# marcin119a/vae-los-angeles

Measured on AMD Instinct MI355X. Metric: training samples/sec, MultiModalVAE batch 65536, higher is better.
Workload: dtype bf16

## Files before the change

### include/mmvae_hip.h

```cpp
#ifndef MMVAE_HIP_H
#define MMVAE_HIP_H
#include <stdint.h>

#ifdef __cplusplus
extern "C" {
#endif

#define MMVAE_OK 0
#define MMVAE_ERR_ARG (-1)
#define MMVAE_ERR_DTYPE (-2)

enum { MMVAE_F32 = 0, MMVAE_BF16 = 1 };
enum { MMVAE_PREC_F32 = 0, MMVAE_PREC_BF16 = 1 };
enum { MMVAE_PRO_NONE = 0, MMVAE_PRO_BN_RELU_DROP = 1, MMVAE_PRO_BN_BWD_APPLY = 2 };
enum { MMVAE_EPI_STORE = 0, MMVAE_EPI_RELU_MASK = 1, MMVAE_EPI_BN_BWD = 2, MMVAE_EPI_LOSS_MSE = 3, MMVAE_EPI_LOSS_BCE_LOGIT = 4 };
enum { MMVAE_ACT_NONE = 0, MMVAE_ACT_RELU = 1, MMVAE_ACT_SIGMOID = 2 };

#define MMVAE_TILE 128

int mmvae_abi_version(void);
int mmvae_set_tuning(int32_t key, int32_t value);

typedef struct {
    const float* src; void* dst;
// ... 87 lines not shown
} mmvae_fuse_fwd_args;
int mmvae_fuse_reparam_fwd(const mmvae_fuse_fwd_args* args, void* stream);

typedef struct {
    int32_t B, L, n_mod;
    const float* g_mu; const float* g_lv;
    const float* dz; const float* dz2; const float* dz3; int64_t lddz;
    const float* eps; const float* logvar;
    float* d_heads; int64_t ld_heads;
    float* d_table; const int64_t* site; int32_t S;
    void* d_heads_lp; int64_t ld_heads_lp;
    int32_t table_copies;
} mmvae_fuse_bwd_args;
#define MMVAE_TABLE_COPIES 8
int mmvae_fuse_reparam_bwd(const mmvae_fuse_bwd_args* args, void* stream);

int mmvae_embed_proj_fwd(int32_t S, int32_t E, int32_t L, const float* emb, const float* w, const float* b, float* table, void* stream);
int mmvae_embed_proj_bwd(int32_t S, int32_t E, int32_t L, const float* emb, const float* w, const float* d_table, int32_t table_copies,
                         float* d_emb, float* d_w, float* d_b, void* stream);
typedef struct {
    int32_t B, L, n_mod;
    const float* head; int64_t ld_head;
    const float* table; const int64_t* site; int32_t S;
    float* latent;
    void* z; int32_t z_dtype; int64_t ldz;
} mmvae_fuse_mean_fwd_args;
int mmvae_fuse_mean_fwd(const mmvae_fuse_mean_fwd_args* args, void* stream);
typedef struct {
    int32_t B, L, n_mod;
    const float* dz; int64_t lddz;
    const float* g_latent;
    float* d_head; int64_t ld_head;
    void* d_head_lp; int64_t ld_head_lp;
    float* d_table; const int64_t* site; int32_t S; int32_t table_copies;
} mmvae_fuse_mean_bwd_args;
int mmvae_fuse_mean_bwd(const mmvae_fuse_mean_bwd_args* args, void* stream);

typedef struct {
    const void* y; int64_t ldy; int32_t K;
    const float* scale; const float* shift;
    const uint8_t* mask; int64_t ld_mask; float inv_keep;
    const void* finalize;
    const void* w; int64_t ldw; const float* bias;
} mmvae_latent_enc;
typedef struct {
    int32_t prec, B, L, n_mod;
    mmvae_latent_enc enc_a, enc_b;
    const float* table; const int64_t* site; int32_t S;
    const float* eps;
    float* mu; float* logvar;
    void* z; int64_t ldz;
    const void* w_stem; int64_t ldw_stem; const float* bias_stem; int32_t N_stem;
    void* h0; int64_t ldh0;
} mmvae_latent_fwd_args;
int mmvae_latent_fwd(const mmvae_latent_fwd_args* args, void* stream);

typedef struct {
    int32_t prec, B, L, n_mod;
    mmvae_latent_enc enc;
    const float* table; const int64_t* site; int32_t S;
    float* latent;
    void* z; int64_t ldz;
    const void* w_stem; int64_t ldw_stem; const float* bias_stem; int32_t N_stem;
    void* h0; int64_t ldh0;
} mmvae_ae_latent_fwd_args;
int mmvae_ae_latent_fwd(const mmvae_ae_latent_fwd_args* args, void* stream);

typedef struct {
    int32_t prec, B, S, L, hidden;
    const void* h0; int64_t ldh0;
    const void* w; int64_t ldw; const void* wt; int64_t ldwt; const float* bias;
    const int64_t* site; const float* class_weights;
    const float* mu; const float* logvar;
    float beta, gamma; const float* beta_gamma_dev;
    double* sums;
    float* g_c; int64_t ld_gc;
    void* d0; int64_t ldd0;
    float* g_mu; float* g_lv;
} mmvae_class_tail_args;
int mmvae_class_tail(const mmvae_class_tail_args* args, void* stream);
int mmvae_class_tail_fits(int32_t prec, int32_t S, int32_t hidden, int32_t L, int64_t ldh0, int64_t ldd0);

typedef struct {
    int32_t prec, B, G, N, K, act;
    const void* a; int64_t lda;
    const void* w; int64_t ldw; const float* bias;
    float* mean; int64_t ld_mean;
    float* std; int64_t ld_std;
} mmvae_group_moments_args;
int mmvae_gemm_nt_group_moments(const mmvae_group_moments_args* args, void* stream);
int mmvae_gemm_nt_group_moments_fits(int32_t prec, int32_t B, int32_t G, int32_t N, int32_t K, int32_t act, int32_t with_std,
                                     int64_t lda, int64_t ldw);

typedef struct {
    int32_t B, A, D, S, L;
    const float* recon_a; const void* a; int64_t ld_ra, ld_a;
    const float* recon_b; const void* b; int64_t ld_rb, ld_b;
    const float* logits; int64_t ld_logits; const int64_t* site; const float* class_weights;
    const float* mu; const float* logvar;
    float beta, gamma;
    double* sums;
    void* g_a; int32_t g_a_dtype; int64_t ld_ga;
    void* g_b; int32_t g_b_dtype; int64_t ld_gb; int32_t grad_b_wrt_logit;
    float* g_c; int64_t ld_gc;
    float* g_mu; float* g_lv;
    const float* beta_gamma_dev;
    int32_t a_dtype, b_dtype;
} mmvae_loss_args;
int mmvae_vae_loss(const mmvae_loss_args* args, void* stream);
int mmvae_loss_finalize(const double* sums, float beta, float gamma, const float* beta_gamma_dev, float* out5, void* stream);

int mmvae_sigmoid_bwd(int32_t M, int32_t N, const float* g, int64_t ldg, const float* p, int64_t ldpp,
                      void* out, int32_t out_dtype, int64_t ldo, void* stream);

int mmvae_scale_if_needed(void* x, int32_t dtype, int64_t n, const float* scale_dev, void* stream);
#define MMVAE_SCALE_MAX 8
typedef struct { void* x; int64_t n; int32_t dtype; int32_t pad_; } mmvae_scale_item;
int mmvae_scale_many(const mmvae_scale_item* items_host, int32_t n_items, const float* scale_dev, void* stream);

#define MMVAE_CTR_COPIES 16384
int mmvae_noise(uint8_t* mask, int64_t n_mask, float keep_prob, float* eps, int64_t n_eps, uint64_t seed, uint64_t offset,
                uint64_t* offset_dev, int32_t advance, void* stream);
int mmvae_counter_add(uint64_t* counter_dev, uint64_t inc, void* stream);

#define MMVAE_HEAD_ZERO_MAX 4
typedef struct {
    int32_t S, E, L, n_zero;
    const float* emb; const float* w_mu; const float* b_mu; const float* w_lv; const float* b_lv; float* table;
    void* zero_ptr[MMVAE_HEAD_ZERO_MAX]; int64_t zero_bytes[MMVAE_HEAD_ZERO_MAX];
    const mmvae_prep_item* prep_items; int32_t n_prep;
    int32_t advance;
    uint8_t* mask; int64_t n_mask; float* eps; int64_t n_eps;
    uint64_t seed, offset; uint64_t* offset_dev; float keep_prob; int32_t pad_;
} mmvae_step_head_args;
int mmvae_step_head(const mmvae_step_head_args* args, void* stream);

#define MMVAE_GATHER_MAX 4
typedef struct { const void* src; void* dst; int64_t src_row_stride; int64_t dst_row_stride; int32_t row_bytes; int32_t pad_; } mmvae_gather_item;
int mmvae_gather_rows(const mmvae_gather_item* items_host, int32_t n_items, const int64_t* idx_dev, int32_t rows,
                      int64_t src_rows, void* stream);

int mmvae_rows_to_bf16(const void* src, int32_t src_dtype, int64_t ld_src, void* dst, int64_t ld_dst, int32_t rows, int32_t cols,
                       void* stream);

typedef struct {
    int32_t M, N;
    const void* pred; int32_t pred_dtype; int64_t ld_pred;
    const void* target; int32_t target_dtype; int64_t ld_target;
    const float* col_shift;
    double* col_acc;
    float* row_pearson; float* row_cosine;
} mmvae_metrics_args;
int mmvae_recon_metrics(const mmvae_metrics_args* args, void* stream);

#define MMVAE_KNN_MAXK 96
typedef struct {
    const void* q; const void* t; const float* shift;
    int32_t* idx; float* dist2; void* work;
    int64_t ld_q, ld_t, ld_idx, ld_dist2, work_bytes;
    int32_t Mq, Nt, F, k, q_dtype, t_dtype;
} mmvae_knn_args;
int mmvae_knn_search(const mmvae_knn_args* args, void* stream);
int mmvae_knn_work_bytes(int32_t Mq, int32_t Nt, int32_t k, int64_t* bytes);
int mmvae_knn_splits(int32_t Mq, int32_t Nt, int32_t* splits, int32_t* rows_per_split);

int mmvae_knn_search_l1(const mmvae_knn_args* args, void* stream);
// ... 126 lines not shown
```

### vae-los-angeles_amd/csrc/class_tail.hip

```cpp
#include "common.h"
#include "mmvae_hip.h"
#include "loss_terms.h"
#include "wave_slab.h"

namespace mm {

constexpr int CT_WAVES = 8, CT_THREADS = 64 * CT_WAVES;
constexpr int CT_SP = 32;
constexpr int CT_HID = 64;
constexpr int CT_KU = 6;
constexpr int CT_WROW = 2 * CT_HID + 16;
constexpr int CT_TROW = 2 * CT_SP + 16;
constexpr int CT_XLD = CT_SP + 4;
constexpr int CT_OFF_WT = CT_SP * CT_WROW;
constexpr int CT_OFF_BIAS = CT_OFF_WT + CT_HID * CT_TROW;
constexpr int CT_OFF_CW = CT_OFF_BIAS + CT_SP * 4;
constexpr int CT_OFF_RED = CT_OFF_CW + CT_SP * 4;
constexpr int CT_OFF_SCR = CT_OFF_RED + CT_WAVES * 3 * 8;
constexpr int CT_SCR_E = 16 * CT_XLD * 4;
constexpr int CT_SCR_G = 2 * CT_SCR_E;
constexpr int CT_SCR = CT_SCR_G + 16 * CT_TROW;
constexpr int CT_LDS = CT_OFF_SCR + CT_WAVES * CT_SCR;
static_assert(CT_OFF_SCR % 16 == 0 && CT_SCR % 16 == 0 && CT_SCR_E % 16 == 0, "16-byte LDS vectors");

struct CtArgs {
    int B, S, L, nslabs;
    const bf16* h0; long ldh; const bf16* w; long ldw; const bf16* wt; long ldwt; const float* bias;
    const long long* site; const float* cw; const float* mu; const float* lv;
    float beta, gamma; const float* bg; double* sums;
    float* gc; long ldgc; bf16* d0; long ldd; float* gmu; float* glv;
};

__global__ __launch_bounds__(CT_THREADS) void class_tail_kernel(const CtArgs a) {
    extern __shared__ __attribute__((aligned(16))) unsigned char smem[];
    const int tid = threadIdx.x, lane = tid & 63, wid = tid >> 6;
    const int li = lane & 15, lg = lane >> 4;
    float* const sbias = (float*)(smem + CT_OFF_BIAS);
    float* const scw = (float*)(smem + CT_OFF_CW);
    double* const red = (double*)(smem + CT_OFF_RED);
    unsigned char* const scr = smem + CT_OFF_SCR + wid * CT_SCR;
    float* const sx = (float*)scr;
    float* const sexp = (float*)(scr + CT_SCR_E);
    unsigned char* const sg = scr + CT_SCR_G;
    float beta = a.beta, gamma = a.gamma;
    if (a.bg) { beta = a.bg[0]; gamma = a.bg[1]; }
    const int S = a.S, L = a.L, total = a.B * L;

    bf16x8 hn[2];
    long long yn = 0;
    float mun[CT_KU] = {}, lvn[CT_KU] = {};
    auto fetch = [&](int slab) __attribute__((always_inline)) {
        const int row = min(slab * 16 + li, a.B - 1);
        const bf16* hp = a.h0 + (long)row * a.ldh + 8 * lg;
        hn[0] = *(const bf16x8*)hp;
        hn[1] = *(const bf16x8*)(hp + 32);
        yn = a.site[row];
#pragma unroll
        for (int i = 0; i < CT_KU; ++i) {
            if (64 * i >= 16 * L) break;
            const int idx = min(slab * 16 * L + lane + 64 * i, total - 1);
            mun[i] = a.mu[idx]; lvn[i] = a.lv[idx];
        }
    };

    const int nw = gridDim.x * CT_WAVES;
    int slab = blockIdx.x * CT_WAVES + wid;
    if (slab < a.nslabs) fetch(slab);

    stage_rows<CT_THREADS>(smem, CT_WROW, a.w, a.ldw, CT_SP, 8, tid, EpiCols<false>::wrow);
    stage_rows<CT_THREADS>(smem + CT_OFF_WT, CT_TROW, a.wt, a.ldwt, CT_HID, 4, tid, EpiCols<true>::wrow);
    if (tid < CT_SP) {
        sbias[tid] = (a.bias && tid < S) ? a.bias[tid] : 0.f;
        scw[tid] = (a.cw && tid < S) ? a.cw[tid] : 1.f;
    }
    __syncthreads();

    double dcls = 0.0, dkl = 0.0;
    float nbad = 0.f;
    const int vpr = S >> 2;
    for (; slab < a.nslabs; slab += nw) {
        const bf16x8 hv[2] = {hn[0], hn[1]};
        const long long yl = yn;
        float mu[CT_KU], lv[CT_KU];
#pragma unroll
        for (int i = 0; i < CT_KU; ++i) { mu[i] = mun[i]; lv[i] = lvn[i]; }
        if (slab + nw < a.nslabs) fetch(slab + nw);
        const int row = slab * 16 + li;
        const bool rok = row < a.B;

        f32x4 x[2];
#pragma unroll
        for (int n = 0; n < 2; ++n) {
            f32x4 acc = {0.f, 0.f, 0.f, 0.f};
#pragma unroll
            for (int j = 0; j < 2; ++j) {
                const bf16x8 wf = *(const bf16x8*)(smem + (16 * n + li) * CT_WROW + (4 * j + lg) * 16);
                Mma<bf16>::mma(acc, wf, hv[j]);
            }
            x[n] = acc + *(const f32x4*)(sbias + 16 * n + 4 * lg);
        }
        float m = -INFINITY;
#pragma unroll
        for (int n = 0; n < 2; ++n)
#pragma unroll
            for (int j = 0; j < 4; ++j) {
                if (16 * n + 4 * lg + j >= S) x[n][j] = -INFINITY;
                m = fmaxf(m, x[n][j]);
            }
        m = fmaxf(m, __shfl_xor(m, 16, 64));
        m = fmaxf(m, __shfl_xor(m, 32, 64));
        f32x4 e[2];
#pragma unroll
        for (int n = 0; n < 2; ++n) {
#pragma unroll
            for (int j = 0; j < 4; ++j) e[n][j] = (16 * n + 4 * lg + j < S) ? ce_exp(x[n][j], m) : 0.f;
            *(f32x4*)(sx + li * CT_XLD + 16 * n + 4 * lg) = x[n];
            *(f32x4*)(sexp + li * CT_XLD + 16 * n + 4 * lg) = e[n];
        }
        wave_lds_sync();
        float se = 0.f;
#pragma unroll
        for (int c = 0; c < CT_SP / 4; ++c) {
            const f32x4 v = *(const f32x4*)(sexp + li * CT_XLD + 4 * c);
#pragma unroll
            for (int j = 0; j < 4; ++j) se += v[j];
        }
        const CeLabel lb = ce_label(yl, S, scw);
        const float xy = sx[li * CT_XLD + lb.y];
        if (lg == 0 && rok) {
            dcls += (double)ce_term(lb.w, m, se, xy);
            if (lb.bad) nbad += 1.f;
        }
        const float gw = gamma * lb.w;
        f32x4 g[2];
#pragma unroll
        for (int n = 0; n < 2; ++n)
#pragma unroll
            for (int j = 0; j < 4; ++j) {
                const int c = 16 * n + 4 * lg + j;
                g[n][j] = c < S ? ce_grad(gw, e[n][j], se, c == lb.y) : 0.f;
            }
        wave_lds_sync();
#pragma unroll
        for (int n = 0; n < 2; ++n) {
            *(f32x4*)(sx + li * CT_XLD + 16 * n + 4 * lg) = g[n];
            const bf16x4 gb = {(bf16)g[n][0], (bf16)g[n][1], (bf16)g[n][2], (bf16)g[n][3]};
            *(bf16x4*)(sg + li * CT_TROW + (16 * n + 4 * lg) * 2) = gb;
        }
        wave_lds_sync();
#pragma unroll
        for (int it = 0; it < 2; ++it) {
            const int v = lane + 64 * it;
            const int r = v / vpr, c4 = v - r * vpr;
            if (v < 16 * vpr && slab * 16 + r < a.B)
                *(f32x4*)(a.gc + (long)(slab * 16 + r) * a.ldgc + 4 * c4) = *(const f32x4*)(sx + r * CT_XLD + 4 * c4);
        }
        const bf16x8 gf = *(const bf16x8*)(sg + li * CT_TROW + lg * 16);
        f32x4 acc[4];
#pragma unroll
        for (int q = 0; q < 4; ++q) {
            const bf16x8 wf = *(const bf16x8*)(smem + CT_OFF_WT + (16 * q + li) * CT_TROW + lg * 16);
            acc[q] = f32x4{0.f, 0.f, 0.f, 0.f};
            Mma<bf16>::mma(acc[q], wf, gf);
        }
        uint32_t pk[2][4];
#pragma unroll
        for (int h = 0; h < 2; ++h) {
#pragma unroll
            for (int qd = 0; qd < 4; ++qd) {
                const f32x4 v = qd < 2 ? acc[2 * h] : acc[2 * h + 1];
                const int e0 = 2 * qd;
                const float o0 = (float)hv[h][e0] > 0.f ? v[2 * (qd & 1)] : 0.f;
                const float o1 = (float)hv[h][e0 + 1] > 0.f ? v[2 * (qd & 1) + 1] : 0.f;
                const bf16x2 t = {(bf16)o0, (bf16)o1};
                pk[h][qd] = __builtin_bit_cast(uint32_t, t);
            }
        }
        SWAP_HALVES(pk, li < 8, st0, st1);
        const int rbase = slab * 16 + (li & 7);
        bf16* const crow = line_col(a.d0 + (long)rbase * a.ldd, li, lg);
        if (rbase < a.B) *(uint4*)crow = uint4{st0[0], st0[1], st0[2], st0[3]};
        if (rbase + 8 < a.B) *(uint4*)(crow + 8 * a.ldd) = uint4{st1[0], st1[1], st1[2], st1[3]};

#pragma unroll
        for (int i = 0; i < CT_KU; ++i) {
            if (64 * i >= 16 * L) break;
            const int idx = slab * 16 * L + lane + 64 * i;
            if (lane + 64 * i < 16 * L && idx < total) {
                float gm, gl;
                dkl += (double)kl_elem(mu[i], lv[i], beta, gm, gl);
                a.gmu[idx] = gm; a.glv[idx] = gl;
            }
        }
        wave_lds_sync();
    }

    const double vc = wave_sum_f64(dcls), vk = wave_sum_f64(dkl);
    const float vb = wave_sum(nbad);
    if (lane == 0) { red[wid * 3] = vc; red[wid * 3 + 1] = vk; red[wid * 3 + 2] = (double)vb; }
    __syncthreads();
    if (tid < 3) {
        double v = 0.0;
#pragma unroll
        for (int w = 0; w < CT_WAVES; ++w) v += red[w * 3 + tid];
        if (v != 0.0) unsafeAtomicAdd(a.sums + 2 + tid, v);
    }
}

}

extern "C" int mmvae_class_tail_fits(int32_t prec, int32_t S, int32_t hidden, int32_t L, int64_t ldh0, int64_t ldd0) {
    using namespace mm;
    if (!g_tuning.class_tail_on) return MMVAE_ERR_ARG;
    if (prec != MMVAE_PREC_BF16) return MMVAE_ERR_ARG;
    if (hidden != CT_HID || S < 4 || S > CT_SP || S % 4 || L < 1 || 16 * L > 64 * CT_KU) return MMVAE_ERR_ARG;
    if (ldh0 % 8 || ldh0 < CT_HID || ldd0 % 64 || ldd0 < CT_HID) return MMVAE_ERR_ARG;
    return 0;
}

extern "C" int mmvae_class_tail(const mmvae_class_tail_args* a, void* stream) {
    using namespace mm;
    if (!a) return MMVAE_ERR_ARG;
    { const int rc = mmvae_class_tail_fits(a->prec, a->S, a->hidden, a->L, a->ldh0, a->ldd0); if (rc) return rc; }
    const long wide = a->L > a->S ? a->L : a->S;
    if (a->B <= 0 || (long)a->B * wide >= (1L << 31)) return MMVAE_ERR_ARG;
    if (!a->h0 || !a->w || !a->wt || !a->bias || !a->site || !a->mu || !a->logvar || !a->sums || !a->g_c || !a->d0 || !a->g_mu || !a->g_lv)
        return MMVAE_ERR_ARG;
    if (((uintptr_t)a->h0 & 15) || ((uintptr_t)a->d0 & 127) || ((uintptr_t)a->w & 15) || ((uintptr_t)a->wt & 15)) return MMVAE_ERR_ARG;
    if (a->ldw % 8 || a->ldw < CT_HID || a->ldwt % 8 || a->ldwt < CT_SP) return MMVAE_ERR_ARG;
    if (((uintptr_t)a->g_c & 15) || a->ld_gc % 4 || a->ld_gc < a->S) return MMVAE_ERR_ARG;
    CtArgs k{};
    k.B = a->B; k.S = a->S; k.L = a->L; k.nslabs = (a->B + 15) / 16;
    k.h0 = (const bf16*)a->h0; k.ldh = a->ldh0; k.w = (const bf16*)a->w; k.ldw = a->ldw; k.wt = (const bf16*)a->wt; k.ldwt = a->ldwt;
    k.bias = a->bias; k.site = (const long long*)a->site; k.cw = a->class_weights; k.mu = a->mu; k.lv = a->logvar;
    k.beta = a->beta; k.gamma = a->gamma; k.bg = a->beta_gamma_dev; k.sums = a->sums;
    k.gc = a->g_c; k.ldgc = a->ld_gc; k.d0 = (bf16*)a->d0; k.ldd = a->ldd0; k.gmu = a->g_mu; k.glv = a->g_lv;
    return launch_lds<class_tail_kernel>(dim3(persistent_grid(k.nslabs, CT_WAVES)), dim3(CT_THREADS), CT_LDS, (hipStream_t)stream, k);
}
```

### vae-los-angeles_amd/csrc/common.h

```cpp
#pragma once
#include <hip/hip_runtime.h>
#include <stdint.h>
#include "mmvae_hip.h"

namespace mm {

typedef __bf16 bf16;
typedef __attribute__((ext_vector_type(8))) __bf16 bf16x8;
typedef __attribute__((ext_vector_type(4))) __bf16 bf16x4;
typedef __attribute__((ext_vector_type(2))) __bf16 bf16x2;
typedef __attribute__((ext_vector_type(4))) float f32x4;
typedef __attribute__((ext_vector_type(2))) float f32x2;
typedef __attribute__((ext_vector_type(4))) short s16x4;

constexpr int WAVE = 64;
constexpr int TILE = 128;
constexpr int NTHREADS = 256;
constexpr int ROW_BYTES = 128;
constexpr int NUM_CU = 256;

template <typename CT> struct Mma;

template <> struct Mma<bf16> {
    static constexpr int EPC = 8;
// ... 59 lines not shown
}

struct Philox {
    static __device__ __forceinline__ void round(uint32_t (&c)[4], uint32_t k0, uint32_t k1) {
        const uint32_t M0 = 0xD2511F53u, M1 = 0xCD9E8D57u;
        const uint64_t p0 = (uint64_t)M0 * (uint64_t)c[0], p1 = (uint64_t)M1 * (uint64_t)c[2];
        const uint32_t hi0 = (uint32_t)(p0 >> 32), lo0 = (uint32_t)p0, hi1 = (uint32_t)(p1 >> 32), lo1 = (uint32_t)p1;
        uint32_t n0 = hi1 ^ c[1] ^ k0, n2 = hi0 ^ c[3] ^ k1;
        c[0] = n0; c[1] = lo1; c[2] = n2; c[3] = lo0;
    }
    static __device__ __forceinline__ void gen(uint64_t seed, uint64_t ctr_lo, uint64_t ctr_hi, uint32_t (&out)[4]) {
        uint32_t c[4] = {(uint32_t)ctr_lo, (uint32_t)(ctr_lo >> 32), (uint32_t)ctr_hi, (uint32_t)(ctr_hi >> 32)};
        uint32_t k0 = (uint32_t)seed, k1 = (uint32_t)(seed >> 32);
#pragma unroll
        for (int i = 0; i < 10; ++i) { round(c, k0, k1); k0 += 0x9E3779B9u; k1 += 0xBB67AE85u; }
        for (int i = 0; i < 4; ++i) out[i] = c[i];
    }
};

enum StampKernel { STAMP_NT = 0, STAMP_NT2 = 1, STAMP_NTP = 2, STAMP_TN = 3, STAMP_TNW = 4 };
constexpr int STAMP_SLOTS = 16;

#ifdef MM_STAMP
#define STAMP_T(x) unsigned long long x = __builtin_readcyclecounter()
#define STAMP_ADD(i, d) st_acc[i] += (d)
#define STAMP_ONLY(...) __VA_ARGS__
#define UNSTAMPED(...)
#define STAMP_BUFFER(name) \
    __device__ unsigned long long stamps_##name[STAMP_SLOTS]; \
    int stamp_read_##name(uint64_t* out, int n, int reset) { return stamp_copy(HIP_SYMBOL(stamps_##name), out, n, reset); }
#define STAMP_ENTRY() \
    extern "C" int mmvae_debug_stamps(int32_t kernel, uint64_t* out, int32_t n, int32_t reset) { \
        switch (kernel) { \
        case mm::STAMP_NT: return mm::stamp_read_nt(out, n, reset); \
        case mm::STAMP_NT2: return mm::stamp_read_nt2(out, n, reset); \
        case mm::STAMP_NTP: return mm::stamp_read_ntp(out, n, reset); \
        case mm::STAMP_TN: return mm::stamp_read_tn(out, n, reset); \
        case mm::STAMP_TNW: return mm::stamp_read_tnw(out, n, reset); \
        } \
        return MMVAE_ERR_ARG; \
    }

template <int N>
__device__ __forceinline__ void stamp_flush(unsigned long long* slots, const unsigned long long (&acc)[N]) {
#pragma unroll
    for (int i = 0; i < N; ++i) atomicAdd(&slots[i], acc[i]);
}
inline int stamp_copy(const void* sym, uint64_t* out, int n, int reset) {
    if (n < 0 || n > STAMP_SLOTS) return MMVAE_ERR_ARG;
    hipError_t e = hipMemcpyFromSymbol(out, sym, n * sizeof(uint64_t));
    if (e != hipSuccess || !reset) return (int)e;
    const uint64_t z[STAMP_SLOTS] = {};
    return (int)hipMemcpyToSymbol(sym, z, sizeof(z));
}
int stamp_read_nt(uint64_t*, int, int);
int stamp_read_nt2(uint64_t*, int, int);
int stamp_read_ntp(uint64_t*, int, int);
int stamp_read_tn(uint64_t*, int, int);
int stamp_read_tnw(uint64_t*, int, int);
#else
#define STAMP_T(x)
#define STAMP_ADD(i, d)
#define STAMP_ONLY(...)
#define UNSTAMPED(...) __VA_ARGS__
#define STAMP_BUFFER(name)
#define STAMP_ENTRY()
#endif


struct Tuning {
    int nt_wide_min_m = NUM_CU * 128;
    int nt2_on = 1;
    long split_bytes = 1L << 32;
    long block_bytes = 1L << 31;
    int tn_wide_on = 1;
    int bnbwd_stream = 1;
    int relu_stream = 1;
    int ntp_on = 1;
    int ntp_min_m = 16384;
    int latent_on = 1;
    int class_tail_on = 1;
    int step_head_on = 1;
    int ae_latent_on = 1;
    int tn_riders_on = 1;
};
inline Tuning g_tuning;

constexpr int NOT_TAKEN = 1 << 30;

template <auto Kernel, typename... Args>
inline int launch_lds(dim3 grid, dim3 block, int lds, hipStream_t st, const Args&... args) {
    static bool attr_done = false;
    if (!attr_done) {
        hipError_t e = hipFuncSetAttribute((const void*)Kernel, hipFuncAttributeMaxDynamicSharedMemorySize, lds);
        if (e != hipSuccess) return (int)e;
        attr_done = true;
    }
    hipLaunchKernelGGL(Kernel, grid, block, lds, st, args...);
    return (int)hipGetLastError();
}

inline bool needs_row_blocks(long M, long row_bytes) { return M * row_bytes >= g_tuning.split_bytes; }

template <typename F>
inline int for_row_blocks(long M, long row_bytes, F&& block) {
    long rows = g_tuning.block_bytes / row_bytes;
    if (rows <= 0) return MMVAE_ERR_ARG;
    const long nblk = (M + rows - 1) / rows;
    long even = (M + nblk - 1) / nblk;
    if (even >= 256) even = (even + 255) & ~255L;
    if (even <= rows) rows = even;
    else if (rows >= 256) rows &= ~255L;
    for (long r0 = 0; r0 < M; r0 += rows) {
        const int rc = block(r0, (int)(M - r0 < rows ? M - r0 : rows));
        if (rc) return rc;
    }
    return 0;
}

struct SplitPlan { int nsplit, rps; };
inline SplitPlan plan_splits(int M, int MT, int want, int ntiles, int wg_target, int limit = 0) {
    int nsplit = want;
    if (want <= 0) {
        nsplit = wg_target / ntiles;
        if (nsplit >= 8) nsplit &= ~7;
    }
    if (want <= 0 || limit > 0) {
        const int max_split = (M + 4 * MT - 1) / (4 * MT);
        if (nsplit > max_split) nsplit = max_split;
        if (limit > 0 && nsplit > limit) nsplit = limit;
        if (nsplit < 1) nsplit = 1;
    }
    int rps = (M + nsplit - 1) / nsplit;
    rps = (rps + MT - 1) / MT * MT;
    return {(M + rps - 1) / rps, rps};
}

inline int vec_width(long ld, long n, const void* p, long esize = 4) {
    const uintptr_t a = (uintptr_t)p;
    if (ld % 4 == 0 && n % 4 == 0 && (a & (4 * esize - 1)) == 0) return 4;
    if (ld % 2 == 0 && n % 2 == 0 && (a & (2 * esize - 1)) == 0) return 2;
    return 1;
}

}

#define MM_CHECK_LAUNCH() do { hipError_t e_ = hipGetLastError(); if (e_ != hipSuccess) return (int)e_; } while (0)
```

### vae-los-angeles_amd/csrc/gemm_nt.hip

```cpp
#include "common.h"
#include "mmvae_hip.h"
#include "gemm_src.h"
#include "gemm_nt_epi.h"
#include "gemm_nt2.h"

namespace mm {

STAMP_BUFFER(nt)

__device__ __forceinline__ int swz(int row, int chunk) { return row * ROW_BYTES + ((chunk ^ (row & 7)) << 4); }

template <int WN> struct NtLds {
    static constexpr int BUF = (TILE + 64 * WN) * ROW_BYTES;
    static constexpr int STAGE = 2 * BUF;
    static constexpr int ECOL = STAGE + 4096 + 4 * 64 * WN * 4;
    static constexpr int TOTAL = ECOL + 8 * 64 * WN * 4;
};

template <typename CT, typename Src, typename Epi, int WN>
__global__ __launch_bounds__(128 * WN, 2)
void gemm_nt_kernel(Src src, const CT* __restrict__ W, long ldw, int M, int N, int K, int gx, int gy, Epi epi)
{
    constexpr int EPC = Mma<CT>::EPC;
    constexpr int BK = ROW_BYTES / (int)sizeof(CT);
// ... 228 lines not shown
        EpiBnBwd<LP, LP> e{(LP*)a->c, a->ldc, (const LP*)a->h, a->ldh, a->epi_mask, a->ld_epi_mask,
                           a->bn_scale, a->bn_shift, a->bn_mean, a->bn_rstd, a->epi_inv_keep, a->bn_coef, a->bn_phase,
                           a->bn_phase == 1 ? nullptr : a->stat1, a->bn_phase == 1 ? nullptr : a->stat2};
        return launch_nt<CT>(src, a->w, a->ldw, a->M, a->N, a->K, e, st);
    }
    case MMVAE_EPI_LOSS_MSE:
    case MMVAE_EPI_LOSS_BCE_LOGIT: {
        if constexpr (sizeof(CT) == 2 && is_plain_bf16<Src>) {
            if (!a->h || !a->c || !a->stat1 || a->c_dtype != MMVAE_BF16 || a->accumulate || a->K <= 64) return MMVAE_ERR_ARG;
            const bool h16 = a->h_dtype == MMVAE_BF16;
            if (a->h_dtype != MMVAE_F32 && !h16) return MMVAE_ERR_DTYPE;
            const long hsz = h16 ? 2 : 4;
            if (a->ldc % 8 || ((uintptr_t)a->c & 15) || ((uintptr_t)a->h & (hsz - 1))) return MMVAE_ERR_ARG;
            if ((long)a->M * a->ldh * hsz >= (1L << 40)) return MMVAE_ERR_ARG;
            const int vt = vec_width(a->ldh, a->N, a->h, hsz);
            const bool mse = a->epilogue == MMVAE_EPI_LOSS_MSE;
#define MM_LOSS_EPI(MODE, VT, TT) { EpiLoss<MODE, VT, TT> e{(bf16*)a->c, a->ldc, (const TT*)a->h, a->ldh, a->bias, a->stat1}; \
                                    return launch_nt2<EpiLoss<MODE, VT, TT>, 2>(src.p, src.lda, a->w, a->ldw, a->M, a->N, a->K, e, st); }
#define MM_LOSS_VT(MODE, TT) { if (vt == 4) MM_LOSS_EPI(MODE, 4, TT) if (vt == 2) MM_LOSS_EPI(MODE, 2, TT) MM_LOSS_EPI(MODE, 1, TT) }
            if (h16) { if (mse) MM_LOSS_VT(0, bf16) MM_LOSS_VT(1, bf16) }
            if (mse) MM_LOSS_VT(0, float)
            MM_LOSS_VT(1, float)
#undef MM_LOSS_VT
#undef MM_LOSS_EPI
        }
        return MMVAE_ERR_ARG;
    }
    }
    return MMVAE_ERR_ARG;
}

BnFin bn_fin_of(const mmvae_gemm_nt_args* a) {
    return bn_fin_from((const mmvae_bn_finalize_args*)a->pro_finalize);
}
static bool bn_fin_ok(const mmvae_gemm_nt_args* a) {
    if (!a->pro_finalize) return true;
    const mmvae_bn_finalize_args* b = (const mmvae_bn_finalize_args*)a->pro_finalize;
    return a->prologue == MMVAE_PRO_BN_RELU_DROP && b->N == a->K && b->M >= 2 && b->sum && b->sumsq && b->gamma && b->beta && b->mean && b->rstd && b->scale && b->shift;
}

template <typename CT>
static int dispatch_src(const mmvae_gemm_nt_args* a, hipStream_t st) {
    constexpr int EPC = Mma<CT>::EPC;
    if (a->prologue == MMVAE_PRO_BN_RELU_DROP) {
        if ((a->a_dtype == MMVAE_BF16) != (sizeof(CT) == 2)) return MMVAE_ERR_DTYPE;
        if (a->K > 512 || a->lda % EPC || ((uintptr_t)a->a & 15) || (!a->pro_finalize && (!a->pro_scale || !a->pro_shift))) return MMVAE_ERR_ARG;
        if (a->pro_mask && (a->ld_pro_mask % 4 || ((uintptr_t)a->pro_mask & 3))) return MMVAE_ERR_ARG;
        SrcBnReluDrop<CT> s{(const CT*)a->a, a->lda, a->M, a->K, a->pro_scale, a->pro_shift, a->pro_mask, a->ld_pro_mask, a->pro_inv_keep, bn_fin_of(a)};
        return dispatch_epi<CT>(a, s, st);
    }
    if (a->a_dtype == MMVAE_BF16) {
        if constexpr (sizeof(CT) == 2) {
            if (a->lda % 8 || ((uintptr_t)a->a & 15)) return MMVAE_ERR_ARG;
            SrcPlain<CT, bf16, 8> s{(const bf16*)a->a, a->lda, a->M, a->K};
            return dispatch_epi<CT>(a, s, st);
        }
        return MMVAE_ERR_DTYPE;
    }
    return with_src_f32<CT>(a->a, a->lda, a->M, a->K, [&](const auto& s) { return dispatch_epi<CT>(a, s, st); });
}

}

extern "C" int mmvae_set_tuning(int32_t key, int32_t value) {
    mm::Tuning& t = mm::g_tuning;
    switch (key) {
    case 0: t.nt_wide_min_m = value; return 0;
    case 2: t.nt2_on = value; return 0;
    case 3:
        if (value != 0 && (value < 17 || value > 32)) return MMVAE_ERR_ARG;
        t.split_bytes = value ? 1L << value : mm::Tuning{}.split_bytes;
        t.block_bytes = t.split_bytes / 2;
        return 0;
    case 4: t.tn_wide_on = value; return 0;
    case 6: t.bnbwd_stream = value; return 0;
    case 7: t.relu_stream = value; return 0;
    case 8: t.ntp_on = value; return 0;
    case 9: t.ntp_min_m = value; return 0;
    case 10: t.latent_on = value; return 0;
    case 12: t.class_tail_on = value; return 0;
    case 13: t.step_head_on = value; return 0;
    case 14: t.tn_riders_on = value; return 0;
    case 15: t.ae_latent_on = value; return 0;
    }
    return MMVAE_ERR_ARG;
}

extern "C" int mmvae_gemm_nt(const mmvae_gemm_nt_args* a, void* stream) {
    if (!a || !a->a || !a->w || (!a->c && !(a->epilogue == MMVAE_EPI_BN_BWD && a->bn_phase == 0))) return MMVAE_ERR_ARG;
    if (a->M <= 0 || a->N <= 0 || a->K <= 0) return MMVAE_ERR_ARG;
    if (a->ldw % 64 || ((uintptr_t)a->w & 15)) return MMVAE_ERR_ARG;
    const long lim = 1L << 32;
    if (((long)a->N + 256) * a->ldw * 4 >= lim) return MMVAE_ERR_ARG;
    const long a_row = (long)a->lda * (a->a_dtype == MMVAE_BF16 ? 2 : 4);
    long row_bytes = a_row > (long)a->ld_pro_mask ? a_row : (long)a->ld_pro_mask;
    if (!mm::bn_fin_ok(a)) return MMVAE_ERR_ARG;
    if (mm::needs_row_blocks(a->M, row_bytes)) {
        if (a->pro_finalize || a->pro_out) return MMVAE_ERR_ARG;
        const bool loss_epi = a->epilogue == MMVAE_EPI_LOSS_MSE || a->epilogue == MMVAE_EPI_LOSS_BCE_LOGIT;
        const long hsz = loss_epi ? (a->h_dtype == MMVAE_BF16 ? 2 : 4) : (a->prec == MMVAE_PREC_BF16 ? 2 : 4);
        return mm::for_row_blocks(a->M, row_bytes, [&](long r0, int rows) {
            mmvae_gemm_nt_args s = *a;
            s.M = rows;
            s.a = (const char*)a->a + r0 * a_row;
            if (a->c) s.c = (char*)a->c + r0 * a->ldc * (a->c_dtype == MMVAE_BF16 ? 2 : 4);
            if (a->h) s.h = (const char*)a->h + r0 * a->ldh * hsz;
            if (a->pro_mask) s.pro_mask = a->pro_mask + r0 * a->ld_pro_mask;
            if (a->epi_mask) s.epi_mask = a->epi_mask + r0 * a->ld_epi_mask;
            return mmvae_gemm_nt(&s, stream);
        });
    }
    hipStream_t st = (hipStream_t)stream;
    { const int rc = mm::ntp_dispatch(a, st); if (rc != mm::NOT_TAKEN) return rc; }
    if (a->pro_out) return MMVAE_ERR_ARG;
    if (a->prec == MMVAE_PREC_BF16) return mm::dispatch_src<mm::bf16>(a, st);
    if (a->prec == MMVAE_PREC_F32) return mm::dispatch_src<float>(a, st);
    return MMVAE_ERR_ARG;
}

STAMP_ENTRY()
```

### vae-los-angeles_amd/csrc/latent.hip

```cpp
#include "common.h"
#include "mmvae_hip.h"
#include "gemm_src.h"
#include "fuse_math.h"
#include "wave_slab.h"

namespace mm {

constexpr int LAT_WAVES = 8, LAT_THREADS = 64 * LAT_WAVES;
constexpr int LAT_NK = 8;
constexpr int LAT_HN = 48;
constexpr int LAT_FU = LAT_HN / 2 * 16 / 64;
constexpr int LAT_NS = 448;
constexpr int LAT_MAXTAB = 1024;
constexpr int LAT_WROW = LAT_NK * 64 + 16;
constexpr int LAT_SROW = 64 + 16;
constexpr int LAT_SUMLD = 52;
constexpr int LAT_OFF_WS = 2 * LAT_HN * LAT_WROW;
constexpr int LAT_OFF_AUX = LAT_OFF_WS + LAT_NS * LAT_SROW;
constexpr int LAT_OFF_BIAS = LAT_OFF_AUX + 2 * 4096;
constexpr int LAT_OFF_TAB = LAT_OFF_BIAS + (2 * LAT_HN + LAT_NS) * 4;
constexpr int LAT_OFF_SCR = LAT_OFF_TAB + LAT_MAXTAB * 4;
constexpr int LAT_SCR_Z = 16 * LAT_SUMLD * 4;
constexpr int LAT_SCR = LAT_SCR_Z + 16 * LAT_SROW;
constexpr int LAT_LDS = LAT_OFF_SCR + LAT_WAVES * LAT_SCR;

struct LatEnc { SrcBnReluDrop<bf16> src; const bf16* w; long ldw; const float* bias; int nk; };
struct LatArgs {
    LatEnc e[2];
    int B, L, n_mod, S;
    const float* table; const long long* site; const float* eps; float* mu; float* logvar;
    bf16* z; long ldz;
    const bf16* ws; long ldws; const float* bs; int ns;
    bf16* h0; long ldh0;
    int nslabs;
};

template <bool DET>
__global__ __launch_bounds__(LAT_THREADS) void latent_fwd_kernel(const LatArgs a) {
    typedef SrcBnReluDrop<bf16>::Raw Raw;
    extern __shared__ __attribute__((aligned(16))) unsigned char smem[];
    const int tid = threadIdx.x, lane = tid & 63, wid = tid >> 6;
    const int li = lane & 15, lg = lane >> 4;
    float* const aux = (float*)(smem + LAT_OFF_AUX);
    float* const sbias = (float*)(smem + LAT_OFF_BIAS);
    float* const stab = (float*)(smem + LAT_OFF_TAB);
    unsigned char* const scr = smem + LAT_OFF_SCR + wid * LAT_SCR;
    float* const ssum = (float*)scr;
    unsigned char* const sz = scr + LAT_SCR_Z;
    const int L = a.L, L2 = DET ? a.L : 2 * a.L;
    const bool any_enc = a.e[0].nk + a.e[1].nk > 0;

    int fr[LAT_FU], fl[LAT_FU];
#pragma unroll
    for (int i = 0; i < LAT_FU; ++i) { const int x = lane + 64 * i; fr[i] = x / L; fl[i] = x - fr[i] * L; }
    const int zcpr = (int)(a.ldz >> 3), zr = lane / zcpr, zc = lane - zr * zcpr;
    const float inv_n = 1.f / (float)a.n_mod;
    const int total = a.B * L;

    Raw raw[2][LAT_NK];
    float eps_r[LAT_FU] = {};
    long long site_r[LAT_FU] = {};
    auto fetch = [&](int slab) __attribute__((always_inline)) {
        const int row = slab * 16 + li;
#pragma unroll
        for (int e = 0; e < 2; ++e)
#pragma unroll
            for (int j = 0; j < LAT_NK; ++j)
                if (j < a.e[e].nk) a.e[e].src.fetch(raw[e][j], row, 32 * j + 8 * lg);
        if constexpr (!DET) {
#pragma unroll
            for (int i = 0; i < LAT_FU; ++i) {
                const int idx = min(slab * 16 * L + lane + 64 * i, total - 1);
                eps_r[i] = a.eps[idx];
            }
        }
        if (a.table) {
#pragma unroll
            for (int i = 0; i < LAT_FU; ++i) site_r[i] = a.site[min(slab * 16 + fr[i], a.B - 1)];
        }
    };

    const int nw = gridDim.x * LAT_WAVES;
    int slab = blockIdx.x * LAT_WAVES + wid;
    if (slab < a.nslabs) fetch(slab);

#pragma unroll
    for (int e = 0; e < 2; ++e) {
        if (a.e[e].nk == 0) continue;
        static_assert(NTHREADS <= LAT_THREADS && 32 * LAT_NK <= 512, "SrcBnReluDrop's table: 512 columns, filled by NTHREADS threads");
        if (tid < NTHREADS) a.e[e].src.init(aux + e * 1024, tid, 0);
        stage_rows<LAT_THREADS>(smem + e * LAT_HN * LAT_WROW, LAT_WROW, a.e[e].w, a.e[e].ldw, LAT_HN, a.e[e].nk * 4, tid, EpiCols<false>::wrow);
        if (tid < LAT_HN) sbias[e * LAT_HN + tid] = (a.e[e].bias && tid < L2) ? a.e[e].bias[tid] : 0.f;
    }
    stage_rows<LAT_THREADS>(smem + LAT_OFF_WS, LAT_SROW, a.ws, a.ldws, a.ns, 4, tid, [](int x) { return (x & ~63) + EpiCols<true>::wrow(x & 63); });
    for (int c = tid; c < a.ns; c += LAT_THREADS) sbias[2 * LAT_HN + c] = a.bs ? a.bs[c] : 0.f;
    if (a.table) for (int i = tid; i < a.S * L2; i += LAT_THREADS) stab[i] = a.table[i];
    for (int i = lane; i < 16 * LAT_SROW / 16; i += 64) ((uint4*)sz)[i] = uint4{0u, 0u, 0u, 0u};
    __syncthreads();

    for (; slab < a.nslabs; slab += nw) {
        f32x4 hs[3];
#pragma unroll
        for (int e = 0; e < 2; ++e) {
            if (a.e[e].nk == 0) continue;
            f32x4 acc[3];
#pragma unroll
            for (int n = 0; n < 3; ++n) acc[n] = f32x4{0.f, 0.f, 0.f, 0.f};
#pragma unroll
            for (int j = 0; j < LAT_NK; ++j) {
                if (j >= a.e[e].nk) break;
                Chunk<bf16> o;
                a.e[e].src.finish_fast(raw[e][j], 32 * j + 8 * lg, o, aux + e * 1024);
#pragma unroll
                for (int n = 0; n < 3; ++n) {
                    const bf16x8 wf = *(const bf16x8*)(smem + (e * LAT_HN + 16 * n + li) * LAT_WROW + (4 * j + lg) * 16);
                    Mma<bf16>::mma(acc[n], wf, o.v);
                }
            }
#pragma unroll
            for (int n = 0; n < 3; ++n) {
                const f32x4 h = acc[n] + *(const f32x4*)(sbias + e * LAT_HN + 16 * n + 4 * lg);
                hs[n] = (e == 1 && a.e[0].nk) ? hs[n] + h : h;
            }
        }
        if (any_enc) {
#pragma unroll
            for (int n = 0; n < 3; ++n) *(f32x4*)(ssum + li * LAT_SUMLD + 16 * n + 4 * lg) = hs[n];
        }
        float ep[LAT_FU];
        long long st[LAT_FU];
#pragma unroll
        for (int i = 0; i < LAT_FU; ++i) { ep[i] = eps_r[i]; st[i] = site_r[i]; }
        if (slab + nw < a.nslabs) fetch(slab + nw);
        wave_lds_sync();

#pragma unroll
        for (int i = 0; i < LAT_FU; ++i) {
            if (lane + 64 * i >= 16 * L) break;
            const int r = fr[i], l = fl[i];
            if constexpr (DET) {
                float sum = 0.f;
                bool first = true;
                if (any_enc) { sum = ssum[r * LAT_SUMLD + l]; first = false; }
                if (a.table) {
                    const long long s = st[i];
                    const bool ok = s >= 0 && s < a.S;
                    const float t = ok ? stab[(int)s * L + l] : __builtin_nanf("");
                    sum = first ? t : sum + t;
                }
                const float m = fuse_mean_elem(sum, a.n_mod, inv_n);
                const int idx = slab * 16 * L + lane + 64 * i;
                if (idx < total) a.mu[idx] = m;
                ((bf16*)sz)[r * (LAT_SROW / 2) + l] = (bf16)m;
                continue;
            }
            float mu = 0.f, lv = 0.f;
            if (any_enc) { mu += ssum[r * LAT_SUMLD + l]; lv += ssum[r * LAT_SUMLD + L + l]; }
            if (a.table) {
                const long long s = st[i];
                const bool ok = s >= 0 && s < a.S;
                const int sc = ok ? (int)s : 0;
                const float bad = ok ? 0.f : __builtin_nanf("");
                mu += stab[sc * L2 + l] + bad; lv += stab[sc * L2 + L + l] + bad;
            }
            const float zf = fuse_reparam_elem(mu, lv, a.n_mod, inv_n, ep[i]);
            const int idx = slab * 16 * L + lane + 64 * i;
            if (idx < total) { a.mu[idx] = mu; a.logvar[idx] = lv; }
            ((bf16*)sz)[r * (LAT_SROW / 2) + l] = (bf16)zf;
        }
        wave_lds_sync();
        if (lane < 16 * zcpr && slab * 16 + zr < a.B)
            *(uint4*)(a.z + (long)(slab * 16 + zr) * a.ldz + zc * 8) = *(const uint4*)(sz + zr * LAT_SROW + zc * 16);

        const bf16x8 zf8 = *(const bf16x8*)(sz + li * LAT_SROW + lg * 16);
        const bool lowl = li < 8;
        const int rbase = slab * 16 + (li & 7);
        bf16* const crow = line_col(a.h0 + (long)rbase * a.ldh0, li, lg);
        const bool ok0 = rbase < a.B, ok1 = rbase + 8 < a.B;
        for (int p = 0; p < (a.ns >> 6); ++p) {
            f32x4 acc[4];
#pragma unroll
            for (int q = 0; q < 4; ++q) {
                const bf16x8 wf = *(const bf16x8*)(smem + LAT_OFF_WS + (64 * p + 16 * q + li) * LAT_SROW + lg * 16);
                acc[q] = f32x4{0.f, 0.f, 0.f, 0.f};
                Mma<bf16>::mma(acc[q], wf, zf8);
            }
            uint32_t pk[2][4];
#pragma unroll
            for (int h = 0; h < 2; ++h) {
                const float* bp = sbias + 2 * LAT_HN + 64 * p + 32 * h + 8 * lg;
                const f32x4 b0 = *(const f32x4*)bp, b1 = *(const f32x4*)(bp + 4);
                const f32x4 x0 = acc[2 * h] + b0, x1 = acc[2 * h + 1] + b1;
#pragma unroll
                for (int qd = 0; qd < 4; ++qd) {
                    const f32x4 x = qd < 2 ? x0 : x1;
                    const bf16x2 t = {(bf16)fmaxf(x[2 * (qd & 1)], 0.f), (bf16)fmaxf(x[2 * (qd & 1) + 1], 0.f)};
                    pk[h][qd] = __builtin_bit_cast(uint32_t, t);
                }
            }
            SWAP_HALVES(pk, lowl, st0, st1);
            if (ok0) *(uint4*)(crow + 64 * p) = uint4{st0[0], st0[1], st0[2], st0[3]};
            if (ok1) *(uint4*)(crow + 8 * a.ldh0 + 64 * p) = uint4{st1[0], st1[1], st1[2], st1[3]};
        }
        wave_lds_sync();
    }
}

static int lat_enc(const mmvae_latent_enc& e, int B, LatEnc& o) {
    o = LatEnc{};
    if (!e.y) return 0;
    const mmvae_bn_finalize_args* f = (const mmvae_bn_finalize_args*)e.finalize;
    if (e.K < 32 || e.K % 32 || e.K > 32 * LAT_NK || e.ldy % 8 || e.ldy < e.K || ((uintptr_t)e.y & 15)) return MMVAE_ERR_ARG;
    if (!e.w || e.ldw % 64 || e.ldw < e.K || ((uintptr_t)e.w & 15)) return MMVAE_ERR_ARG;
    if (!f && (!e.scale || !e.shift)) return MMVAE_ERR_ARG;
    if (f && (f->N != e.K || f->M != B || B < 2 || !f->sum || !f->sumsq || !f->gamma || !f->beta || !f->mean || !f->rstd || !f->scale || !f->shift))
        return MMVAE_ERR_ARG;
    if (e.mask && (e.ld_mask % 8 || e.ld_mask < e.K || ((uintptr_t)e.mask & 7))) return MMVAE_ERR_ARG;
    const long lim = 1L << 32;
    if ((long)B * e.ldy * 2 >= lim || (e.mask && (long)B * e.ld_mask >= lim)) return MMVAE_ERR_ARG;
    o.src = SrcBnReluDrop<bf16>{(const bf16*)e.y, e.ldy, B, e.K, e.scale, e.shift, e.mask, e.ld_mask, e.inv_keep, bn_fin_from(f)};
    o.w = (const bf16*)e.w; o.ldw = e.ldw; o.bias = e.bias; o.nk = e.K / 32;
    return 0;
}

template <bool DET, typename A>
static int latent_check_launch(const A& a, bool own_ok, const mmvae_latent_enc& enc_a, const mmvae_latent_enc* enc_b, LatArgs& k, void* stream) {
    if (a.prec != MMVAE_PREC_BF16) return MMVAE_ERR_DTYPE;
    if (a.B <= 0 || a.L <= 0 || (long)a.B * a.L >= (1L << 31) || !own_ok) return MMVAE_ERR_ARG;
    if (!a.z || !a.w_stem || !a.h0) return MMVAE_ERR_ARG;
    const int present = (enc_a.y != nullptr) + (enc_b && enc_b->y != nullptr) + (a.table != nullptr);
    if (present == 0 || present != a.n_mod) return MMVAE_ERR_ARG;
    if (a.table && (!a.site || a.S <= 0)) return MMVAE_ERR_ARG;
    if (a.ldz % 8 || a.ldz < a.L || a.ldz > 32 || ((uintptr_t)a.z & 15)) return MMVAE_ERR_ARG;
    if (a.N_stem < 64 || a.N_stem % 64 || a.N_stem > LAT_NS || a.ldw_stem % 64 || a.ldw_stem < 32 || ((uintptr_t)a.w_stem & 15)) return MMVAE_ERR_ARG;
    if (a.ldh0 % 64 || a.ldh0 < a.N_stem || ((uintptr_t)a.h0 & 127) || (long)a.B * a.ldh0 * 2 >= (1L << 32)) return MMVAE_ERR_ARG;
    { const int rc = lat_enc(enc_a, a.B, k.e[0]); if (rc) return rc; }
    if (enc_b) { const int rc = lat_enc(*enc_b, a.B, k.e[1]); if (rc) return rc; }
    k.B = a.B; k.L = a.L; k.n_mod = a.n_mod; k.S = a.S;
    k.table = a.table; k.site = (const long long*)a.site;
    k.z = (bf16*)a.z; k.ldz = a.ldz;
    k.ws = (const bf16*)a.w_stem; k.ldws = a.ldw_stem; k.bs = a.bias_stem; k.ns = a.N_stem;
    k.h0 = (bf16*)a.h0; k.ldh0 = a.ldh0;
    k.nslabs = (a.B + 15) / 16;
    return launch_lds<latent_fwd_kernel<DET>>(dim3(persistent_grid(k.nslabs, LAT_WAVES)), dim3(LAT_THREADS), LAT_LDS, (hipStream_t)stream, k);
}

}

extern "C" int mmvae_latent_fwd(const mmvae_latent_fwd_args* a, void* stream) {
    using namespace mm;
    if (!a || !g_tuning.latent_on) return MMVAE_ERR_ARG;
    const bool own_ok = 2 * a->L <= LAT_HN && a->eps && a->mu && a->logvar && (!a->table || (long)a->S * 2 * a->L <= LAT_MAXTAB);
    LatArgs k{};
    k.eps = a->eps; k.mu = a->mu; k.logvar = a->logvar;
    return latent_check_launch<false>(*a, own_ok, a->enc_a, &a->enc_b, k, stream);
}

extern "C" int mmvae_ae_latent_fwd(const mmvae_ae_latent_fwd_args* a, void* stream) {
    using namespace mm;
    if (!a || !g_tuning.ae_latent_on) return MMVAE_ERR_ARG;
    const bool own_ok = a->L <= LAT_HN / 2 && a->latent && (!a->table || (long)a->S * a->L <= LAT_MAXTAB);
    LatArgs k{};
    k.mu = a->latent;
    return latent_check_launch<true>(*a, own_ok, a->enc, nullptr, k, stream);
}
```

### vae-los-angeles_amd/mmvae/_lib.py

```python
import ctypes as C
import os

_HERE = os.path.dirname(os.path.abspath(__file__))
LIB_PATH = os.environ.get("MMVAE_LIB_PATH") or os.path.join(_HERE, "libmmvae_hip.so")
ABI_VERSION = 20

F32, BF16 = 0, 1
PREC_F32, PREC_BF16 = 0, 1
PRO_NONE, PRO_BN_RELU_DROP, PRO_BN_BWD_APPLY = 0, 1, 2
TABLE_COPIES = 8
EPI_STORE, EPI_RELU_MASK, EPI_BN_BWD, EPI_LOSS_MSE, EPI_LOSS_BCE_LOGIT = 0, 1, 2, 3, 4
ACT_NONE, ACT_RELU, ACT_SIGMOID = 0, 1, 2
TILE = 128
TN_GROUP_MAX = 8
KNN_MAXK = 96
SIL_MAXC = 64
PCA_MAXK = 64
LN_MAXN = 1024
WCE_MAXC = 64
STD_MAX_PARTS = 4
CTR_COPIES = 16384

i32, i64, f32, vp = C.c_int32, C.c_int64, C.c_float, C.c_void_p

# ... 33 lines not shown


class TnRiders(C.Structure):
    _fields_ = [("S", i32), ("E", i32), ("L", i32), ("table_copies", i32),
                ("emb", vp), ("w_mu", vp), ("w_lv", vp), ("d_table", vp),
                ("d_emb", vp), ("d_w_mu", vp), ("d_b_mu", vp), ("d_w_lv", vp), ("d_b_lv", vp),
                ("sums", vp), ("beta", f32), ("gamma", f32), ("beta_gamma_dev", vp), ("out5", vp)]


HEAD_ZERO_MAX = 4


class StepHeadArgs(C.Structure):
    _fields_ = [("S", i32), ("E", i32), ("L", i32), ("n_zero", i32),
                ("emb", vp), ("w_mu", vp), ("b_mu", vp), ("w_lv", vp), ("b_lv", vp), ("table", vp),
                ("zero_ptr", vp * HEAD_ZERO_MAX), ("zero_bytes", i64 * HEAD_ZERO_MAX),
                ("prep_items", vp), ("n_prep", i32),
                ("advance", i32),
                ("mask", vp), ("n_mask", i64), ("eps", vp), ("n_eps", i64),
                ("seed", C.c_uint64), ("offset", C.c_uint64), ("offset_dev", vp), ("keep_prob", f32), ("pad_", i32)]


class ScaleItem(C.Structure):
    _fields_ = [("x", vp), ("n", i64), ("dtype", i32), ("pad_", i32)]


class BnFinalizeArgs(C.Structure):
    _fields_ = [("M", i32), ("N", i32), ("sum", vp), ("sumsq", vp),
                ("gamma", vp), ("beta", vp), ("eps", f32), ("momentum", f32),
                ("running_mean", vp), ("running_var", vp), ("num_batches_tracked", vp),
                ("mean", vp), ("rstd", vp), ("scale", vp), ("shift", vp)]


class BnBwdFinalizeArgs(C.Structure):
    _fields_ = [("M", i32), ("N", i32), ("sum_d", vp), ("sum_dx", vp),
                ("gamma", vp), ("rstd", vp), ("dgamma", vp), ("dbeta", vp), ("coef", vp), ("eval_mode", i32)]


class FuseFwdArgs(C.Structure):
    _fields_ = [("B", i32), ("L", i32), ("n_mod", i32),
                ("heads_a", vp), ("heads_b", vp), ("ld_heads", i64),
                ("table", vp), ("site", vp), ("S", i32),
                ("eps", vp), ("mu", vp), ("logvar", vp),
                ("z", vp), ("z_dtype", i32), ("ldz", i64)]


class LatentEnc(C.Structure):
    _fields_ = [("y", vp), ("ldy", i64), ("K", i32), ("scale", vp), ("shift", vp),
                ("mask", vp), ("ld_mask", i64), ("inv_keep", f32), ("finalize", vp),
                ("w", vp), ("ldw", i64), ("bias", vp)]


class LatentFwdArgs(C.Structure):
    _fields_ = [("prec", i32), ("B", i32), ("L", i32), ("n_mod", i32),
                ("enc_a", LatentEnc), ("enc_b", LatentEnc),
                ("table", vp), ("site", vp), ("S", i32),
                ("eps", vp), ("mu", vp), ("logvar", vp),
                ("z", vp), ("ldz", i64),
                ("w_stem", vp), ("ldw_stem", i64), ("bias_stem", vp), ("N_stem", i32),
                ("h0", vp), ("ldh0", i64)]


class AELatentFwdArgs(C.Structure):
    _fields_ = [("prec", i32), ("B", i32), ("L", i32), ("n_mod", i32),
                ("enc", LatentEnc),
                ("table", vp), ("site", vp), ("S", i32),
                ("latent", vp),
                ("z", vp), ("ldz", i64),
                ("w_stem", vp), ("ldw_stem", i64), ("bias_stem", vp), ("N_stem", i32),
                ("h0", vp), ("ldh0", i64)]


class ClassTailArgs(C.Structure):
    _fields_ = [("prec", i32), ("B", i32), ("S", i32), ("L", i32), ("hidden", i32),
                ("h0", vp), ("ldh0", i64),
                ("w", vp), ("ldw", i64), ("wt", vp), ("ldwt", i64), ("bias", vp),
                ("site", vp), ("class_weights", vp),
                ("mu", vp), ("logvar", vp),
                ("beta", f32), ("gamma", f32), ("beta_gamma_dev", vp),
                ("sums", vp),
                ("g_c", vp), ("ld_gc", i64),
                ("d0", vp), ("ldd0", i64),
                ("g_mu", vp), ("g_lv", vp)]


class GroupMomentsArgs(C.Structure):
    _fields_ = [("prec", i32), ("B", i32), ("G", i32), ("N", i32), ("K", i32), ("act", i32),
                ("a", vp), ("lda", i64),
                ("w", vp), ("ldw", i64), ("bias", vp),
                ("mean", vp), ("ld_mean", i64),
                ("std", vp), ("ld_std", i64)]


class FuseBwdArgs(C.Structure):
    _fields_ = [("B", i32), ("L", i32), ("n_mod", i32),
                ("g_mu", vp), ("g_lv", vp), ("dz", vp), ("dz2", vp), ("dz3", vp), ("lddz", i64),
                ("eps", vp), ("logvar", vp),
                ("d_heads", vp), ("ld_heads", i64),
                ("d_table", vp), ("site", vp), ("S", i32), ("d_heads_lp", vp), ("ld_heads_lp", i64), ("table_copies", i32)]


class FuseMeanFwdArgs(C.Structure):
    _fields_ = [("B", i32), ("L", i32), ("n_mod", i32),
                ("head", vp), ("ld_head", i64),
                ("table", vp), ("site", vp), ("S", i32),
                ("latent", vp),
                ("z", vp), ("z_dtype", i32), ("ldz", i64)]


class FuseMeanBwdArgs(C.Structure):
    _fields_ = [("B", i32), ("L", i32), ("n_mod", i32),
                ("dz", vp), ("lddz", i64),
                ("g_latent", vp),
                ("d_head", vp), ("ld_head", i64),
                ("d_head_lp", vp), ("ld_head_lp", i64),
                ("d_table", vp), ("site", vp), ("S", i32), ("table_copies", i32)]


class LossArgs(C.Structure):
    _fields_ = [("B", i32), ("A", i32), ("D", i32), ("S", i32), ("L", i32),
                ("recon_a", vp), ("a", vp), ("ld_ra", i64), ("ld_a", i64),
                ("recon_b", vp), ("b", vp), ("ld_rb", i64), ("ld_b", i64),
                ("logits", vp), ("ld_logits", i64), ("site", vp), ("class_weights", vp),
                ("mu", vp), ("logvar", vp),
                ("beta", f32), ("gamma", f32),
                ("sums", vp),
                ("g_a", vp), ("g_a_dtype", i32), ("ld_ga", i64),
                ("g_b", vp), ("g_b_dtype", i32), ("ld_gb", i64), ("grad_b_wrt_logit", i32),
                ("g_c", vp), ("ld_gc", i64),
                ("g_mu", vp), ("g_lv", vp), ("beta_gamma_dev", vp), ("a_dtype", i32), ("b_dtype", i32)]


class MetricsArgs(C.Structure):
    _fields_ = [("M", i32), ("N", i32),
                ("pred", vp), ("pred_dtype", i32), ("ld_pred", i64),
                ("target", vp), ("target_dtype", i32), ("ld_target", i64),
                ("col_shift", vp), ("col_acc", vp), ("row_pearson", vp), ("row_cosine", vp)]


class KnnArgs(C.Structure):
    _fields_ = [("q", vp), ("t", vp), ("shift", vp), ("idx", vp), ("dist2", vp), ("work", vp),
                ("ld_q", i64), ("ld_t", i64), ("ld_idx", i64), ("ld_dist2", i64), ("work_bytes", i64),
                ("Mq", i32), ("Nt", i32), ("F", i32), ("k", i32), ("q_dtype", i32), ("t_dtype", i32)]


class KnnGroupArgs(C.Structure):
    _fields_ = [("base", KnnArgs), ("q_same", vp), ("t_same", vp), ("q_differ", vp), ("t_differ", vp), ("metric", i32)]


class SilhouetteArgs(C.Structure):
    _fields_ = [("x", vp), ("shift", vp), ("order", vp), ("class_start", vp), ("s", vp), ("intra", vp), ("inter", vp), ("work", vp),
                ("ld_x", i64), ("work_bytes", i64),
                ("N", i32), ("F", i32), ("C", i32), ("splits", i32), ("x_dtype", i32), ("pad_", i32)]


class PcaScatterArgs(C.Structure):
    _fields_ = [("x", vp), ("shift", vp), ("s", vp), ("work", vp),
                ("ld_x", i64), ("ld_s", i64), ("work_bytes", i64),
                ("N", i32), ("F", i32), ("splits", i32), ("x_dtype", i32)]


class PcaProjectArgs(C.Structure):
    _fields_ = [("x", vp), ("shift", vp), ("v", vp), ("y", vp),
                ("ld_x", i64), ("ld_v", i64), ("ld_y", i64),
                ("N", i32), ("F", i32), ("k", i32), ("x_dtype", i32)]

# ... 6 lines not shown
    _fields_ = [("part", StdPart * STD_MAX_PARTS),
                ("mean", vp), ("var", vp), ("scale", vp), ("work", vp),
                ("work_bytes", i64),
                ("rows", i32), ("n_parts", i32), ("splits", i32), ("pad_", i32)]


class StandardizeApplyArgs(C.Structure):
    _fields_ = [("part", StdPart * STD_MAX_PARTS),
                ("mean", vp), ("scale", vp), ("z", vp),
                ("ldz", i64),
                ("rows", i32), ("n_parts", i32)]


class TsneAffinitiesArgs(C.Structure):
    _fields_ = [("dist2", vp), ("p", vp), ("beta", vp),
                ("ld_dist2", i64), ("ld_p", i64),
                ("N", i32), ("k", i32), ("perplexity", f32), ("pad_", i32)]


class TsneGradientArgs(C.Structure):
    _fields_ = [("y", vp), ("row_ptr", vp), ("col", vp), ("val", vp), ("grad", vp), ("z", vp), ("err", vp), ("z_row", vp), ("work", vp),
                ("nnz", i64), ("work_bytes", i64),
                ("N", i32), ("splits", i32), ("exaggeration", f32), ("pad_", i32)]


class TsneUpdateArgs(C.Structure):
    _fields_ = [("y", vp), ("update", vp), ("gains", vp), ("grad", vp), ("grad_norm", vp), ("work", vp),
                ("work_bytes", i64),
                ("N", i32), ("momentum", f32), ("learning_rate", f32), ("pad_", i32)]


class LnActFwdArgs(C.Structure):
    _fields_ = [("z", vp), ("gamma", vp), ("beta", vp), ("mask", vp), ("y", vp), ("mean", vp), ("rstd", vp),
                ("ldz", i64), ("ld_mask", i64), ("ldy", i64),
                ("M", i32), ("N", i32), ("layer_norm", i32), ("eps", f32), ("inv_keep", f32), ("pad_", i32)]


class LnActBwdArgs(C.Structure):
    _fields_ = [("dy", vp), ("z", vp), ("mean", vp), ("rstd", vp), ("gamma", vp), ("beta", vp), ("mask", vp),
                ("dz", vp), ("dgamma", vp), ("dbeta", vp), ("work", vp),
                ("lddy", i64), ("ldz", i64), ("ld_mask", i64), ("lddz", i64), ("work_bytes", i64),
                ("M", i32), ("N", i32), ("layer_norm", i32), ("inv_keep", f32)]


class WceArgs(C.Structure):
    _fields_ = [("logits", vp), ("labels", vp), ("class_weights", vp), ("sums", vp), ("g", vp), ("pred", vp), ("nll", vp), ("confusion", vp),
                ("ld", i64), ("ldg", i64),
                ("M", i32), ("C", i32)]


class GatherItem(C.Structure):
    _fields_ = [("src", vp), ("dst", vp), ("src_row_stride", i64), ("dst_row_stride", i64), ("row_bytes", i32), ("pad_", i32)]


class AdamWItem(C.Structure):
    _fields_ = [("p", vp), ("g", vp), ("m", vp), ("v", vp), ("n", i64)]


_SIGNATURES = {
    "mmvae_set_tuning": [i32, i32],
    "mmvae_prep_weights": [vp, i32, vp],
    "mmvae_gemm_nt": [C.POINTER(GemmNtArgs), vp],
    "mmvae_gemm_tn": [C.POINTER(GemmTnArgs), vp],
    "mmvae_gemm_tn_group": [vp, i32, vp],
    "mmvae_gemm_tn_group_riders": [vp, i32, C.POINTER(TnRiders), vp],
    "mmvae_step_head": [C.POINTER(StepHeadArgs), vp],
    "mmvae_bn_finalize": [C.POINTER(BnFinalizeArgs), vp],
    "mmvae_bn_eval_coeffs": [i32, vp, vp, vp, vp, f32, vp, vp, vp, vp, vp],
    "mmvae_bn_bwd_finalize": [C.POINTER(BnBwdFinalizeArgs), vp],
    "mmvae_bn_bwd_apply": [i32, i32, i32, vp, i64, vp, i64, vp, vp, vp, vp],
    "mmvae_bn_bwd_finalize_apply": [i32, i32, i32, vp, i64, vp, i64, vp, vp, vp, vp, vp, vp, vp, i32, vp],
    "mmvae_embed_table_fwd": [i32, i32, i32, vp, vp, vp, vp, vp, vp, vp],
    "mmvae_embed_table_bwd": [i32, i32, i32, vp, vp, vp, vp, i32, vp, vp, vp, vp, vp, vp],
    "mmvae_fuse_reparam_fwd": [C.POINTER(FuseFwdArgs), vp],
    "mmvae_fuse_reparam_bwd": [C.POINTER(FuseBwdArgs), vp],
    "mmvae_embed_proj_fwd": [i32, i32, i32, vp, vp, vp, vp, vp],
    "mmvae_embed_proj_bwd": [i32, i32, i32, vp, vp, vp, i32, vp, vp, vp, vp],
    "mmvae_fuse_mean_fwd": [C.POINTER(FuseMeanFwdArgs), vp],
    "mmvae_fuse_mean_bwd": [C.POINTER(FuseMeanBwdArgs), vp],
    "mmvae_latent_fwd": [C.POINTER(LatentFwdArgs), vp],
    "mmvae_ae_latent_fwd": [C.POINTER(AELatentFwdArgs), vp],
    "mmvae_class_tail": [C.POINTER(ClassTailArgs), vp],
    "mmvae_class_tail_fits": [i32, i32, i32, i32, i64, i64],
    "mmvae_gemm_nt_group_moments": [C.POINTER(GroupMomentsArgs), vp],
    "mmvae_gemm_nt_group_moments_fits": [i32, i32, i32, i32, i32, i32, i32, i64, i64],
    "mmvae_vae_loss": [C.POINTER(LossArgs), vp],
    "mmvae_loss_finalize": [vp, f32, f32, vp, vp, vp],
    "mmvae_recon_metrics": [C.POINTER(MetricsArgs), vp],
    "mmvae_knn_search": [C.POINTER(KnnArgs), vp],
    "mmvae_knn_work_bytes": [i32, i32, i32, C.POINTER(i64)],
    "mmvae_knn_splits": [i32, i32, C.POINTER(i32), C.POINTER(i32)],
    "mmvae_knn_mean_rows": [vp, i64, vp, i32, i64, vp, i64, i32, i32, i32, i32, vp],
    "mmvae_knn_search_l1": [C.POINTER(KnnArgs), vp],
    "mmvae_knn_l1_work_bytes": [i32, i32, i32, C.POINTER(i64)],
    "mmvae_knn_weighted_rows": [vp, i64, vp, i64, i32, vp, i32, i64, vp, i64, i32, i32, i32, i32, vp],
    "mmvae_knn_search_grouped": [C.POINTER(KnnGroupArgs), vp],
    "mmvae_knn_group_work_bytes": [i32, i32, i32, i32, C.POINTER(i64)],
    "mmvae_silhouette_samples": [C.POINTER(SilhouetteArgs), vp],
    "mmvae_silhouette_work_bytes": [i32, i32, i32, C.POINTER(i64)],
    "mmvae_silhouette_splits": [i32, i32, i32, C.POINTER(i32)],
    "mmvae_pca_scatter": [C.POINTER(PcaScatterArgs), vp],
    "mmvae_pca_scatter_splits": [i32, i32, i32, C.POINTER(i32)],
    "mmvae_pca_scatter_work_bytes": [i32, i32, i32, C.POINTER(i64)],
    "mmvae_pca_project": [C.POINTER(PcaProjectArgs), vp],
    "mmvae_standardize_fit": [C.POINTER(StandardizeFitArgs), vp],
    "mmvae_standardize_fit_splits": [i32, i64, i32, C.POINTER(i32)],
    "mmvae_standardize_fit_work_bytes": [i32, i64, i32, C.POINTER(i64)],
    "mmvae_standardize_apply": [C.POINTER(StandardizeApplyArgs), vp],
    "mmvae_tsne_affinities": [C.POINTER(TsneAffinitiesArgs), vp],
    "mmvae_tsne_gradient": [C.POINTER(TsneGradientArgs), vp],
    "mmvae_tsne_gradient_splits": [i32, i32, C.POINTER(i32)],
    "mmvae_tsne_gradient_work_bytes": [i32, i32, C.POINTER(i64)],
    "mmvae_tsne_update": [C.POINTER(TsneUpdateArgs), vp],
    "mmvae_tsne_update_work_bytes": [i32, C.POINTER(i64)],
    "mmvae_ln_act_fwd": [C.POINTER(LnActFwdArgs), vp],
    "mmvae_ln_act_bwd": [C.POINTER(LnActBwdArgs), vp],
    "mmvae_ln_act_bwd_work_bytes": [i32, i32, i32, C.POINTER(i64)],
    "mmvae_wce_mean": [C.POINTER(WceArgs), vp],
    "mmvae_gather_rows": [vp, i32, vp, i32, i64, vp],
    "mmvae_rows_to_bf16": [vp, i32, i64, vp, i64, i32, i32, vp],
    "mmvae_sigmoid_bwd": [i32, i32, vp, i64, vp, i64, vp, i32, i64, vp],
    "mmvae_scale_if_needed": [vp, i32, i64, vp, vp],
    "mmvae_scale_many": [C.POINTER(ScaleItem), i32, vp, vp],
    "mmvae_noise": [vp, i64, f32, vp, i64, C.c_uint64, C.c_uint64, vp, i32, vp],
    "mmvae_counter_add": [vp, C.c_uint64, vp],
    "mmvae_adamw_step": [vp, i32, f32, f32, f32, f32, f32, f32, f32, i32, vp, i32, vp, vp],
    "mmvae_adam_step": [vp, i32, f32, f32, f32, f32, f32, f32, f32, i32, vp, i32, vp, vp],
}
EXPORTED = ["mmvae_abi_version"] + sorted(_SIGNATURES)

_lib = None


class MMVAELibraryError(RuntimeError):
    pass


class MMVAEArgError(RuntimeError):
    """The library refused the arguments (MMVAE_ERR_ARG / MMVAE_ERR_DTYPE) and enqueued nothing (mmvae_hip.h)."""


def load():
    global _lib
    if _lib is not None:
        return _lib
    if not os.path.exists(LIB_PATH):
        raise MMVAELibraryError(
            f"{LIB_PATH} not found: the HIP extension is required (no CPU / eager fallback). "
            "Build it with `python __graft_entry__.py` or `make -C vae-los-angeles_amd/csrc`.")
    lib = C.CDLL(LIB_PATH)
    lib.mmvae_abi_version.restype = C.c_int
    v = lib.mmvae_abi_version()
    if v != ABI_VERSION:
        raise MMVAELibraryError(f"libmmvae_hip.so ABI {v} != binding ABI {ABI_VERSION}; rebuild")
    for name, argtypes in _SIGNATURES.items():
        fn = getattr(lib, name)
        fn.restype = C.c_int
        fn.argtypes = argtypes
    _lib = lib
    return lib


def check(status, what):
    if status in (-1, -2):
        kind = "invalid argument" if status == -1 else "dtype not supported for this precision"
        raise MMVAEArgError(f"{what} failed: {kind}")
# ... 3 lines not shown
```

### vae-los-angeles_amd/mmvae/engine.py

```python
import os
from dataclasses import dataclass
from typing import NamedTuple, Optional

import torch

from . import ops
from . import _lib as L_
from .ops import (PREC_BF16, PREC_F32, ACT_NONE, ACT_RELU, ACT_SIGMOID, EPI_RELU_MASK, EPI_BN_BWD, DROP_P,
                  ceil_to, act_dtype, Prologue, BnBwdEpilogue, BnBwdFinalize, BnBwdApply)

_PRECISIONS = {"bf16": PREC_BF16, "fp32": PREC_F32, "f32": PREC_F32}
_default_precision = _PRECISIONS[os.environ.get("MMVAE_PRECISION", "bf16").lower()]
_TINY_DW_MAX = 16384


def set_default_precision(name):
    global _default_precision
    _default_precision = _PRECISIONS[name.lower()]


def default_precision():
    return _default_precision


# ... 72 lines not shown
        raise RuntimeError(f"{name}: expected shape (B, {cols}), got {tuple(x.shape)}")
    if not x.is_cuda:
        raise RuntimeError(f"{name}: the MI355X path needs CUDA/HIP tensors (got {x.device}); there is no CPU fallback")
    if x.dtype == torch.bfloat16:
        if prec != PREC_BF16:
            return x.float()
        return x if ops.is_bf16_rows(x) else ops.to_bf16_rows(x)
    if x.dtype != torch.float32:
        x = x.float()
    if x.stride(1) != 1:
        x = x.contiguous()
    return x


def zeros_pack(device, specs, fill=True):
    offs, total = [], 0
    for n, dt in specs:
        offs.append(total)
        total += ceil_to(n * _ITEMSIZE[dt], 16)
    buf = (torch.zeros if fill else torch.empty)(max(total, 16), dtype=torch.uint8, device=device)
    out = [buf[o:o + n * _ITEMSIZE[dt]].view(dt) for o, (n, dt) in zip(offs, specs)]
    return out if fill else (out, buf)


_ITEMSIZE = {torch.float32: 4, torch.float64: 8, torch.uint8: 1, torch.int64: 8}


def carve_arena(flat, params):
    views, off = {}, 0
    for p in params:
        views[p] = flat[off:off + p.numel()].view(p.shape)
        off += p.numel()
    return views


class PrepCache:

    def __init__(self):
        self.key = self.prep = None

    def ensure(self, prec, device, params, build, run=True):
        key = (prec, str(device)) + tuple(p.data_ptr() for p in params)
        if key != self.key:
            pls = build(prec, device)
            self.prep = ops.WeightPrep(pls, device) if pls else None
            self.key = key
        if run and self.prep is not None:
            self.prep.run()
        return self.prep


class BNState:

    def __init__(self, N, device):
        self.buf = torch.empty(4, N, dtype=torch.float32, device=device)
        self.mean, self.rstd, self.scale, self.shift = self.buf[0], self.buf[1], self.buf[2], self.buf[3]


class LayerSave(NamedTuple):
    q: torch.Tensor
    q_prologue: Optional[Prologue]
    y: torch.Tensor
    bn: BNState
    y_prologue: Prologue


class FusedRecon(NamedTuple):
    sums: torch.Tensor
    out5: torch.Tensor
    g: dict
    targets: dict


@dataclass(slots=True, eq=False)
class LossGrads:
    g_outs: list
    g_mu: torch.Tensor
    g_lv: torch.Tensor
    unit_grad: bool
    scale: Optional[torch.Tensor] = None
    armed: bool = False


@dataclass(slots=True, eq=False)
class ClassTail:
    index: int
    head: object
    h0: torch.Tensor
    d0: torch.Tensor
    d0_slice: torch.Tensor
    name: str
    done: bool = False

    def logits(self, prec):
        out = torch.empty(self.h0.shape[0], self.head.N, dtype=torch.float32, device=self.h0.device)
        ops.gemm_nt(prec, self.h0, self.head.w, self.head.N, self.head.K, out, bias=self.head.bias, act=ACT_NONE, tag=f"{self.name}.L1.fwd")
        return out


@dataclass(slots=True, eq=False)
class StepZeros:
    fwd_stats: list
    loss_ws: Optional[tuple]
    arena: Optional[torch.Tensor]
    bwd_stats: list
    d_table: Optional[torch.Tensor]
    unfilled: Optional[torch.Tensor] = None


@dataclass(slots=True, eq=False)
class StepState:
    prec: int
    B: int
    train: bool
    eps: Optional[torch.Tensor] = None
    logvar: Optional[torch.Tensor] = None
    n_mod: int = 0
    enc_a: Optional[list] = None
    enc_b: Optional[list] = None
    site: Optional[torch.Tensor] = None
    dec: Optional[list] = None
    zeros: Optional[StepZeros] = None
    fused: Optional[FusedRecon] = None
    loss_grads: Optional[LossGrads] = None
    class_tail: Optional[ClassTail] = None
    tail_riders: bool = False
    loss_tail: Optional[tuple] = None
    consumed: bool = False


class EncoderMLP:

    def __init__(self, linears, bns, fc_mu, fc_logvar=None, name="enc"):
        self.linears, self.bns, self.fc_mu, self.fc_logvar = list(linears), list(bns), fc_mu, fc_logvar
        self.in_dim = self.linears[0].in_features
        self.latent = fc_mu.out_features
        self.head_width = self.latent * (1 if fc_logvar is None else 2)
        self.name = name

    def prepare(self, prec, device):
        self.pl = [ops.PreparedLinear([l.weight], [l.bias], prec, device) for l in self.linears]
        heads = [self.fc_mu] if self.fc_logvar is None else [self.fc_mu, self.fc_logvar]
        self.pl_heads = ops.PreparedLinear([h.weight for h in heads], [h.bias for h in heads], prec, device)
        return self.pl + [self.pl_heads]

    def params(self):
        out = []
        for l, bn in zip(self.linears, self.bns):
            out += [l.weight, l.bias, bn.weight, bn.bias]
        if self.fc_logvar is None:
            return out + [self.fc_mu.weight, self.fc_mu.bias]
        out += [self.fc_mu.weight, self.fc_logvar.weight, self.fc_mu.bias, self.fc_logvar.bias]
        return out

    def widths(self):
        return [l.out_features for l in self.linears]

    def _consume(self, prec, h, pro, fin, N, K, out, bias, w, tag, stats=None, pro_out=None):
        if fin is not None:
            try:
                ops.gemm_nt(prec, h, w, N, K, out, bias=bias, prologue=pro, stats=stats, tag=tag, pro_out=pro_out, pro_finalize=fin)
                return pro_out
            except L_.MMVAEArgError:
                pass
            ops.bn_finalize_launch(fin)
        try:
            ops.gemm_nt(prec, h, w, N, K, out, bias=bias, prologue=pro, stats=stats, tag=tag, pro_out=pro_out)
            return pro_out
        except L_.MMVAEArgError:
            if pro_out is None:
                raise
            ops.gemm_nt(prec, h, w, N, K, out, bias=bias, prologue=pro, stats=stats, tag=tag)
            return None

    def forward(self, prec, x, train, masks, stats_bufs=None, want_bwd=False, heads=True):
        B, dev = x.shape[0], x.device
        adt = act_dtype(prec)
        layers = []
        h, pro = x, None
        fin = None
        for lin, bn, pl in zip(self.linears, self.bns, self.pl):
            N, K = pl.N, pl.K
            y = torch.empty(B, ceil_to(N, 8), dtype=adt, device=dev)
            st = BNState(N, dev)
            h_act = None
            if want_bwd and pro is not None and ops.can_keep_pro_out(prec, B, N, K, h, y) and pro.mask is not None \
                    and pro.mask.stride(0) % 8 == 0 and pro.mask.data_ptr() % 8 == 0:
                h_act = torch.empty(B, K, dtype=torch.bfloat16, device=dev)
            if train:
                stats = stats_bufs[len(layers)] if stats_bufs is not None else torch.zeros(2, N, dtype=torch.float64, device=dev)
                h_act = self._consume(prec, h, pro, fin, N, K, y, pl.bias, pl.w, f"{self.name}.L{len(layers)}.fwd", stats=stats, pro_out=h_act)
                fin = ops.bn_finalize_args(B, N, stats, bn.weight, bn.bias, bn.running_mean, bn.running_var,
                                           bn.num_batches_tracked, st.mean, st.rstd, st.scale, st.shift, bn.eps,
                                           bn.momentum if bn.momentum is not None else 0.1)
                new_pro = Prologue(st.scale, st.shift, masks[len(layers)], 1.0 / (1.0 - DROP_P))
            else:
                ops.gemm_nt(prec, h, pl.w, N, K, y, bias=pl.bias, prologue=pro, tag=f"{self.name}.L{len(layers)}.fwd")
                ops.bn_eval_coeffs(bn.weight, bn.bias, bn.running_mean, bn.running_var, st.scale, st.shift, bn.eps, st.mean, st.rstd)
                new_pro = Prologue(st.scale, st.shift, None, 1.0)
            layers.append(LayerSave(h, pro, y, st, new_pro) if h_act is None else LayerSave(h_act, None, y, st, new_pro))
            h, pro = y, new_pro
        owed = ops.LatentEncoder(h, pro, fin, self.pl_heads)
        return (self.run_heads(prec, owed) if heads else owed), layers

    def run_heads(self, prec, owed):
        heads = torch.empty(owed.y.shape[0], self.head_width, dtype=torch.float32, device=owed.y.device)
        self._consume(prec, owed.y, owed.prologue, owed.fin, self.head_width, self.pl_heads.K, heads, self.pl_heads.bias, self.pl_heads.w,
                      f"{self.name}.heads.fwd")
        return heads
# ... 85 lines not shown
    def __init__(self, linears, final_sigmoid, name="dec"):
        self.linears, self.final_sigmoid = list(linears), final_sigmoid
        self.out_dim = self.linears[-1].out_features
        self.name = name

    def prepare(self, prec, device):
        self.pl = [ops.PreparedLinear([l.weight], [l.bias], prec, device) for l in self.linears]
        return self.pl

    def params(self):
        out = []
        for l in self.linears:
            out += [l.weight, l.bias]
        return out

    def can_fuse_loss(self, prec):
        return prec == ops.PREC_BF16 and len(self.pl) >= 2 and self.pl[-1].K > 64

    def forward(self, prec, z, fused_loss=None, first=None):
        B, dev = z.shape[0], z.device
        adt = act_dtype(prec)
        acts = [z]
        h = z
        if first is not None:
            acts.append(first)
            h = first
        for j, pl in enumerate(self.pl):
            if j == 0 and first is not None:
                continue
            last = j == len(self.pl) - 1
            if last and fused_loss is not None:
                target, acc = fused_loss
                if tuple(target.shape) != (B, pl.N) or target.dtype not in (torch.float32, torch.bfloat16) or target.stride(1) != 1 \
                        or not target.is_cuda:
                    raise ValueError(f"fused reconstruction loss: target must be fp32 or bf16 [{B}, {pl.N}] with unit inner stride, "
                                     f"got {tuple(target.shape)} {target.dtype}")
                out = torch.empty(B, ceil_to(pl.N, 8), dtype=adt, device=dev)
                ops.gemm_nt(prec, h, pl.w, pl.N, pl.K, out, bias=pl.bias, epilogue=ops.EPI_LOSS_BCE_LOGIT if self.final_sigmoid else ops.EPI_LOSS_MSE,
                            h=target, loss_sum=acc, tag=f"{self.name}.L{j}.fwd")
            elif last:
                out = torch.empty(B, pl.N, dtype=torch.float32, device=dev)
                ops.gemm_nt(prec, h, pl.w, pl.N, pl.K, out, bias=pl.bias, act=ACT_SIGMOID if self.final_sigmoid else ACT_NONE, tag=f"{self.name}.L{j}.fwd")
            else:
                out = torch.empty(B, ceil_to(pl.N, 8), dtype=adt, device=dev)
                ops.gemm_nt(prec, h, pl.w, pl.N, pl.K, out, bias=pl.bias, act=ACT_RELU, tag=f"{self.name}.L{j}.fwd")
                acts.append(out)
            h = out
        return h, acts

    def backward(self, prec, acts, out, g_out, g_is_logit_grad, dz, grads, tn=ops.gemm_tn, d0_out=None, dx_done=None):
        B, dev = g_out.shape[0], g_out.device
        adt = act_dtype(prec)
        d = g_out
        if self.final_sigmoid and not g_is_logit_grad:
            dl = torch.empty(B, ceil_to(self.out_dim, 8), dtype=adt, device=dev)
            ops.sigmoid_bwd(g_out, out, dl)
            d = dl
        for j in reversed(range(len(self.pl))):
            pl, lin = self.pl[j], self.linears[j]
            tn(prec, d, acts[j], grads[lin.weight], grads[lin.bias], pl.N, pl.K, tag=f"{self.name}.L{j}.dW")
            if j > 0 and j == len(self.pl) - 1 and dx_done is not None:
                d = dx_done
            elif j > 0:
                d_prev = d0_out if (j == 1 and d0_out is not None) else torch.empty(B, ceil_to(pl.K, 8), dtype=adt, device=dev)
                ops.gemm_nt(prec, d, pl.wt, pl.K, pl.N, d_prev, epilogue=EPI_RELU_MASK, h=acts[j], tag=f"{self.name}.L{j}.dX")
                d = d_prev
            elif d0_out is None:
                ops.gemm_nt(prec, d, pl.wt, pl.K, pl.N, dz, tag=f"{self.name}.L{j}.dX")


class VAEGraph:

    def __init__(self, enc_a=None, enc_b=None, enc_c=None, decoders=()):
        self.enc_a, self.enc_b, self.enc_c = enc_a, enc_b, enc_c
        self.decoders = list(decoders)
        self.blocks = [b for b in (enc_a, enc_b, enc_c) if b is not None] + self.decoders
        self.latent = (enc_a or enc_b or enc_c).latent
        self._prep = PrepCache()
        self.dec_stem = None
        self.noise = GLOBAL_NOISE
        self.grad_sync = None
        self.fused_recon = None
        self.defer_class_head = False
        self.tail_riders = False

    def _late_decoder_params(self):
        out = []
        for d in self.decoders:
            for l in d.linears:
                if l.weight.numel() <= _TINY_DW_MAX:
                    out += [l.weight, l.bias]
        return out

    def param_list(self):
        out = []
        for b in self.blocks:
            if b not in self.decoders:
                out += b.params()
        late = self._late_decoder_params()
        out += late
        ids = {id(p) for p in late}
        for d in self.decoders:
            out += [p for p in d.params() if id(p) not in ids]
        return out

    def early_cut(self):
        return sum(p.numel() for b in self.blocks if b not in self.decoders for p in b.params()) + sum(p.numel() for p in self._late_decoder_params())

    def _prepare(self, prec, device):
        pls = []
        for b in self.blocks:
            pls += b.prepare(prec, device)
        self.dec_stem = None
        decs = self.decoders
        if (len(decs) >= 2 and all(isinstance(d, DecoderMLP) and len(d.linears) >= 2 for d in decs)
                and all(d.linears[0].in_features == decs[0].linears[0].in_features and d.linears[0].out_features % 8 == 0 for d in decs)):
            self.dec_stem = ops.PreparedLinear([d.linears[0].weight for d in decs], [d.linears[0].bias for d in decs], prec, device)
            pls.append(self.dec_stem)
        return pls

    def zero_pack(self, device, has_a, has_b, has_site, fwd, bwd, fill=True):
        widths = (self.enc_a.widths() if has_a else []) + (self.enc_b.widths() if has_b else [])
        n_sums = 2 * sum(widths)
        n_sites = self.enc_c.embedding.weight.shape[0] if has_site else 0
        tab_w = self.enc_c.table_width * self.latent if has_site else 0
        n_tab = n_sites * tab_w * L_.TABLE_COPIES
        both = fwd and bwd
        packed = zeros_pack(device, [
            (n_sums if fwd else 0, torch.float64),
            (5 if both else 0, torch.float64),
            (5 if both else 0, torch.float32),
            (sum(p.numel() for p in self.param_list()) if bwd else 0, torch.float32),
            (n_sums if bwd else 0, torch.float64),
            (max(n_tab, 1) if bwd else 0, torch.float32)], fill)
        (fwd_sums, loss_sums, loss_out5, arena, bwd_sums, d_table), unfilled = packed if not fill else (packed, None)

        def per_layer(sums):
            return [t.view(2, -1) for t in sums.split([2 * w for w in widths])]
        return StepZeros(fwd_stats=per_layer(fwd_sums) if fwd else [],
                         loss_ws=(loss_sums, loss_out5) if both else None,
                         arena=arena if bwd else None,
                         bwd_stats=per_layer(bwd_sums) if bwd else [],
                         d_table=d_table[:n_tab].view(-1, n_sites, tab_w) if bwd and has_site else None,
                         unfilled=unfilled)

    def forward(self, prec, xa, xb, site, train, want_bwd=False):
        ref = xa if xa is not None else (xb if xb is not None else site)
        if not ref.is_cuda or any(p.device != ref.device for p in self.param_list()):
            raise RuntimeError(f"the MI355X path needs inputs and parameters on one CUDA/HIP device (input on {ref.device}); "
                               "there is no CPU fallback")
        with ops.pinned_stream():
            return self._forward(prec, xa, xb, site, train, train and want_bwd)

    def _head_of_step(self, prec, dev, B, has_a, has_b, has_site, train, want_bwd, eps_width, table_args):
        widths_a = self.enc_a.widths() if (train and has_a) else []
        widths_b = self.enc_b.widths() if (train and has_b) else []
        prep = self._prep.ensure(prec, dev, self.param_list(), self._prepare, run=False)
        masks, eps, noise_launch = self.noise.plan(B, widths_a + widths_b, eps_width, dev)
        if eps_width is None and noise_launch is not None and noise_launch[0] is None:
            noise_launch = None
        head = train and noise_launch is not None
        zeros = self.zero_pack(dev, has_a, has_b, has_site, fwd=True, bwd=want_bwd, fill=not head) if train else None
        if head:
            try:
                ops.step_head(noise_launch, prep, [zeros.unfilled], table_args)
            except L_.MMVAEArgError:
                head = False
        if not head:
            if prep is not None:
                prep.run()
            if noise_launch is not None:
                ops.noise(*noise_launch)
            if zeros is not None and zeros.unfilled is not None:
                zeros.unfilled.zero_()
        if zeros is not None:
            zeros.unfilled = None
        return masks, eps, zeros, len(widths_a), head

    draws_eps = True
    flatten_a = False

    def _forward(self, prec, xa, xb, site, train, want_bwd):
        for x, enc in ((xa, self.enc_a), (xb, self.enc_b)):
            if x is not None and enc is None:
                raise RuntimeError(f"{type(self).__name__}: this graph has no encoder for that input")
        ref = xa if xa is not None else (xb if xb is not None else site)
        dev, B = ref.device, ref.shape[0]
        state = StepState(prec, B, train, tail_riders=self.tail_riders and want_bwd)
        enc_out = [None, None]
        table = None
        table_args = self.enc_c.table_args() if (site is not None and self.enc_c.rides) else None
        masks, eps, zeros, n_a, head = self._head_of_step(prec, dev, B, xa is not None, xb is not None, site is not None, train, want_bwd,
                                                          self.latent if self.draws_eps else None, table_args)
        if head and table_args is not None:
            table = table_args[-1]
        if want_bwd:
            state.zeros = zeros
        fuse_latent = self._fuses_latent(prec)
        if xa is not None:
            xa = _check_input(xa.reshape(xa.shape[0], -1) if self.flatten_a else xa, "a", self.enc_a.in_dim, prec)
            enc_out[0], state.enc_a = self.enc_a.forward(prec, xa, train, masks[:n_a] if train else None,
                                                         zeros.fwd_stats[:n_a] if train else None, want_bwd=want_bwd, heads=not fuse_latent)
        if xb is not None:
            xb = _check_input(xb.reshape(xb.shape[0], -1), "b", self.enc_b.in_dim, prec)
            enc_out[1], state.enc_b = self.enc_b.forward(prec, xb, train, masks[n_a:] if train else None,
                                                         zeros.fwd_stats[n_a:] if train else None, want_bwd=want_bwd, heads=not fuse_latent)
        if site is not None:
            if site.dtype != torch.int64:
                site = site.long()
            site = state.site = site.contiguous()
            if table is None:
                table = self.enc_c.table(table_args)
        state.eps = eps
        state.n_mod = (xa is not None) + (xb is not None) + (table is not None)
        latents, z, H0, stem_done, first0 = self._latent_forward(prec, B, dev, enc_out, table, site, eps, fuse_latent, state)
        return (self._decode(prec, B, dev, z, H0, stem_done, state, zeros, want_bwd, site, first0=first0), *latents, state)

    def _fuses_latent(self, prec):
        return self.dec_stem is not None and prec == PREC_BF16

    def _latent_forward(self, prec, B, dev, enc_out, table, site, eps, fused, state):
        Ld, stem = self.latent, self.dec_stem
        heads_a, heads_b = enc_out
        mu = torch.empty(B, Ld, dtype=torch.float32, device=dev)
        logvar = torch.empty(B, Ld, dtype=torch.float32, device=dev)
        z = torch.empty(B, ceil_to(Ld, 8), dtype=act_dtype(prec), device=dev)
        H0 = torch.empty(B, stem.N, dtype=act_dtype(prec), device=dev) if stem is not None else None
        if fused:
            try:
                ops.latent_fwd(prec, B, Ld, heads_a, heads_b, table, site, eps, mu, logvar, z, stem, H0)
            except L_.MMVAEArgError:
                fused = False
                heads_a = self.enc_a.run_heads(prec, heads_a) if heads_a is not None else None
                heads_b = self.enc_b.run_heads(prec, heads_b) if heads_b is not None else None
        if not fused:
            ops.fuse_reparam_fwd(B, Ld, heads_a, heads_b, table, site, eps, mu, logvar, z)
        state.logvar = logvar.detach()
        return (mu, logvar), z, H0, fused, None

    def _decode(self, prec, B, dev, z, H0, stem_done, state, zeros, want_bwd, site, first0=None):
        stem = self.dec_stem
        outs, state.dec = [None] * len(self.decoders), [None] * len(self.decoders)
        order = sorted(range(len(self.decoders)), key=lambda i: -sum(l.weight.numel() for l in self.decoders[i].linears))
        firsts = [None] * len(self.decoders)
        firsts[0] = first0
        if stem is not None:
            if not stem_done:
                ops.gemm_nt(prec, z, stem.w, stem.N, stem.K, H0, bias=stem.bias, act=ACT_RELU, tag="Decoders.L0.fwd")
            off = 0
            for i, d in enumerate(self.decoders):
                firsts[i] = H0[:, off:off + d.linears[0].out_features]
                off += d.linears[0].out_features
        fused = None
        want = self.fused_recon
        if want is not None and any(t is not None and self.decoders[i].can_fuse_loss(prec) for i, t in enumerate(want)):
            fused = state.fused = FusedRecon(*(zeros.loss_ws if want_bwd else ops.loss_workspace(dev)), {}, {})
        tail_i = self._class_tail_index(prec, H0, want, site) if (self.defer_class_head and fused is not None and want_bwd) else None
        for i in order:
            dec = self.decoders[i]
            tgt = want[i] if (fused is not None and want[i] is not None and dec.can_fuse_loss(prec)) else None
            if i == tail_i:
                D0 = torch.empty(B, stem.N, dtype=act_dtype(prec), device=dev)
                off = sum(d.linears[0].out_features for d in self.decoders[:i])
                state.class_tail = ClassTail(i, dec.pl[1], firsts[i], D0, D0[:, off:off + dec.linears[0].out_features], dec.name)
                o = torch.empty(1, dtype=torch.float32, device=dev).expand(B, dec.out_dim)
                acts = [z, firsts[i]]
            elif tgt is not None:
                k = 1 if dec.final_sigmoid else 0
                g, acts = dec.forward(prec, z, fused_loss=(tgt, fused.sums[k:k + 1]), first=firsts[i])
                fused.g[i], fused.targets[i] = g, tgt
                o = torch.empty(1, dtype=torch.float32, device=dev).expand(B, dec.out_dim)
            else:
                o, acts = dec.forward(prec, z, first=firsts[i])
            outs[i] = o
            state.dec[i] = (acts, o.detach())
        return outs

    def _class_tail_index(self, prec, H0, want, site):
        if self.dec_stem is None or site is None or H0 is None:
            return None
        for i, dec in enumerate(self.decoders):
            if want[i] is None and isinstance(dec, DecoderMLP) and len(dec.pl) == 2 and not dec.final_sigmoid \
                    and ops.class_tail_fits(prec, dec.pl[1].N, dec.pl[1].K, self.latent, H0.stride(0), H0.stride(0)):
                return i
        return None

    def backward(self, state, g_outs, g_logit_flags, g_mu, g_lv):
        with ops.pinned_stream():
            return self._backward(state, g_outs, g_logit_flags, g_mu, g_lv)

    def _backward(self, state, g_outs, g_logit_flags, g_mu, g_lv):
        prec, B = state.prec, state.B
        site = state.site
        dev = state.dec[0][1].device
        Ld = self.latent
        zeros, state.zeros = state.zeros, None
        if zeros is None:
            zeros = self.zero_pack(dev, state.enc_a is not None, state.enc_b is not None, site is not None, fwd=False, bwd=True)
        flat = zeros.arena
        grads = carve_arena(flat, self.param_list())
        n_a = len(state.enc_a) if state.enc_a is not None else 0
        dzs = []
        big = max(p.numel() for p in self.param_list())
        slab = torch.empty(min(64 * big, 1 << 25), dtype=torch.float32, device=dev)

        tiny = []

        def tn(prec_, p, q, dw, db, N, K, q_prologue=None, p_prologue=None, tag=None):
            if p_prologue is None and N * K <= _TINY_DW_MAX:
                tiny.append(dict(p=p, q=q, dw=dw, db=db, N=N, K=K, q_prologue=q_prologue))
                return
            ops.gemm_tn(prec_, p, q, dw, db, N, K, q_prologue=q_prologue, p_prologue=p_prologue, slab=slab, tag=tag)

        def flush_tiny(tag, riders=None):
            rode = False
            if tiny:
                need = ops.TN_GROUP_SPLITS * sum(t_["N"] * t_["K"] for t_ in tiny)
                rode = ops.gemm_tn_group(prec, tiny, torch.empty(need, dtype=torch.float32, device=dev), tag=tag, riders=riders)
                tiny.clear()
            return rode
        stem = self.dec_stem if all(g is not None for g in g_outs) else None
        D0, off = None, 0
        tail = state.class_tail
        if stem is not None:
            D0 = tail.d0 if tail is not None else torch.empty(B, stem.N, dtype=act_dtype(prec), device=dev)
        for i, (dec, (acts, out), g, is_logit) in enumerate(zip(self.decoders, state.dec, g_outs, g_logit_flags)):
            n0 = dec.linears[0].out_features if stem is not None else 0
            if g is None:
                off += n0
                continue
            dx_done = tail.d0_slice if (tail is not None and tail.index == i and tail.done) else None
            if stem is not None:
                dec.backward(prec, acts, out, g, is_logit, None, grads, tn, d0_out=D0[:, off:off + n0], dx_done=dx_done)
                off += n0
                continue
            dz = torch.empty(B, Ld, dtype=torch.float32, device=dev)
            dec.backward(prec, acts, out, g, is_logit, dz, grads, tn, dx_done=dx_done)
            dzs.append(dz)
        if stem is not None:
            dz = torch.empty(B, Ld, dtype=torch.float32, device=dev)
            ops.gemm_nt(prec, D0, stem.wt, stem.K, stem.N, dz, tag="Decoders.L0.dX")
            dzs.append(dz)
        if not dzs:
            dzs.append(torch.zeros(B, Ld, dtype=torch.float32, device=dev))
# ... 77 lines not shown
```

### vae-los-angeles_amd/mmvae/functional.py

```python
from typing import NamedTuple

import torch
from torch.autograd.function import once_differentiable

from . import engine, ops
from .ops import ceil_to, act_dtype


class VAEGraphFn(torch.autograd.Function):

    @staticmethod
    def forward(ctx, graph, prec, train, want_bwd, xa, xb, site, *params):
        ctx.set_materialize_grads(False)
        outs, *latents, state = graph.forward(prec, xa, xb, site, train, want_bwd)
        ctx.graph, ctx.saved, ctx.n_out = graph, state, len(outs)
        graph._last_saved = state
        return (*outs, *latents)

    @staticmethod
    @once_differentiable
    def backward(ctx, *gs):
        graph, state, n_out = ctx.graph, ctx.saved, ctx.n_out
        if state.consumed:
            raise RuntimeError("backward through this forward was already run (buffers are not retained)")
# ... 99 lines not shown
    @staticmethod
    def forward(ctx, spec, *tensors):
        ctx.set_materialize_grads(False)
        total, grads = spec(tensors)
        ctx.grads = grads
        return total

    @staticmethod
    @once_differentiable
    def backward(ctx, g):
        scale = g.reshape(1).float().contiguous()
        out = []
        for t in ctx.grads:
            if t is not None:
                ops.scale_if_needed(t, scale)
            out.append(t)
        return (None, *out)


def _tag_of(t):
    return getattr(t, "_mmvae", None) if t is not None else None


def fused_loss(terms, beta, gamma, class_weights=None, unit_grad=False, beta_gamma_dev=None):
    if not next(v[0] for v in terms.values() if v is not None).is_cuda:
        raise RuntimeError("the MI355X loss kernel needs CUDA/HIP tensors; there is no CPU fallback")
    with ops.pinned_stream():
        return _fused_loss(terms, beta, gamma, class_weights, unit_grad, beta_gamma_dev)


def _validate_loss_args(dev, B, ra, a, rb, b, lg, site, mu, lv, class_weights):
    for nm, pred, tgt in (("a", ra, a), ("b", rb, b), ("logvar", mu, lv)):
        if pred is None:
            continue
        if tgt.device != pred.device or pred.device != dev:
            raise RuntimeError(f"vae_loss: '{nm}' tensors are on different devices ({pred.device} vs {tgt.device}); "
                               "the MI355X loss kernel needs all of them on one CUDA/HIP device")
        if pred.dim() != 2 or tuple(tgt.shape) != tuple(pred.shape) or pred.shape[0] != B:
            raise RuntimeError(f"vae_loss: shape mismatch for '{nm}': prediction {tuple(pred.shape)} vs target {tuple(tgt.shape)} (batch {B})")
    if lg is not None:
        if site.device != dev or lg.device != dev:
            raise RuntimeError(f"vae_loss: site labels / logits are on another device ({site.device}, {lg.device}) than {dev}")
        if lg.dim() != 2 or lg.shape[0] != B or site.dim() != 1 or site.shape[0] != B:
            raise RuntimeError(f"vae_loss: site must have shape ({B},) for logits {tuple(lg.shape)}, got {tuple(site.shape)}")
        if site.dtype in (torch.float16, torch.float32, torch.float64, torch.bfloat16, torch.bool):
            raise RuntimeError(f"vae_loss: site labels must be integer class indices, got {site.dtype}")
        if class_weights is not None and class_weights.numel() != lg.shape[1]:
            raise RuntimeError(f"vae_loss: class_weights has {class_weights.numel()} entries for {lg.shape[1]} classes")


def _fused_loss(terms, beta, gamma, class_weights=None, unit_grad=False, beta_gamma_dev=None):
    any_t = next(v[0] for v in terms.values() if v is not None)
    dev, B = any_t.device, any_t.shape[0]
    ra, a = terms.get("a") or (None, None)
    rb, b = terms.get("b") or (None, None)
    lg, site = terms.get("c") or (None, None)
    mu, lv = terms.get("kl") or (None, None)
    _validate_loss_args(dev, B, ra, a, rb, b, lg, site, mu, lv, class_weights)
    if site is not None and site.dtype != torch.int64:
        site = site.long()
    if site is not None:
        site = site.contiguous()
    cw = None if class_weights is None else class_weights.to(device=dev, dtype=torch.float32).contiguous()
    need_grad = torch.is_grad_enabled() and any(t is not None and t.requires_grad for t in (ra, rb, lg, mu, lv))

    fused, fused_idx = None, {}
    placeholders = []
    for key, (r, t) in (("a", (ra, a)), ("b", (rb, b))):
        tg = _tag_of(r)
        fr = tg.state.fused if tg is not None else None
        if fr is not None and tg.kind == "out" and tg.index in fr.g:
            if fr.targets[tg.index].data_ptr() != t.data_ptr() or tuple(fr.targets[tg.index].shape) != tuple(t.shape):
                raise RuntimeError("fused reconstruction loss: the target passed to the loss is not the tensor the forward was given")
            fused, fused_idx[key] = fr, tg.index
            placeholders.append(r)
    if fused is not None and not (torch.is_grad_enabled()):
        raise RuntimeError("fused reconstruction loss needs the training step (gradients enabled)")
    if "a" in fused_idx:
        ra = None
    if "b" in fused_idx:
        rb = None
    tg = _tag_of(lg)
    tail = tg.state.class_tail if (tg is not None and tg.kind == "out") else None
    if tail is not None and (tail.index != tg.index or tail.done):
        tail = None
    lg_real = lg
    if tail is not None:
        lg = None

    def prep(x):
        return None if x is None else (x if (x.dtype == torch.float32 and x.stride(-1) == 1) else x.float().contiguous())

    def prep_target(x):
        return x if (x is not None and x.dtype == torch.bfloat16 and x.stride(-1) == 1) else prep(x)
    ra_, a_, rb_, b_, lg_, mu_, lv_ = (prep(ra), prep_target(a), prep(rb), prep_target(b), prep(lg), prep(mu), prep(lv))
    if mu_ is not None:
        mu_, lv_ = mu_.contiguous(), lv_.contiguous()
    if fused is not None:
        sums, out4 = fused.sums, fused.out5
    else:
        sums = out4 = None

    tags = [_tag_of(t) for t in (ra, rb, lg_real, mu, lv) if t is not None and t.requires_grad] + [_tag_of(t) for t in placeholders]
    state = tags[0].state if tags and all(t is not None and t.state is tags[0].state for t in tags) else None
    if need_grad and state is not None and not state.consumed and state.loss_grads is None:
        if sums is None:
            zeros = state.zeros
            if zeros is not None and zeros.loss_ws is not None:
                (sums, out4), zeros.loss_ws = zeros.loss_ws, None
            else:
                sums, out4 = ops.loss_workspace(dev)
        adt = act_dtype(state.prec)
        g_outs = [None] * len(state.dec)
        for key, i in fused_idx.items():
            g_outs[i] = fused.g[i]
        ga = gb = gc = None
        if ra is not None and ra.requires_grad:
            ga = torch.empty(B, ceil_to(ra.shape[1], 8), dtype=adt, device=dev)
            g_outs[_tag_of(ra).index] = ga
        if rb is not None and rb.requires_grad:
            gb = torch.empty(B, ceil_to(rb.shape[1], 8), dtype=adt, device=dev)
            g_outs[_tag_of(rb).index] = gb
        if lg_real is not None and lg_real.requires_grad:
            gc = torch.empty(B, lg_real.shape[1], dtype=torch.float32, device=dev)
            g_outs[_tag_of(lg_real).index] = gc
        g_mu = torch.empty(B, mu.shape[1], dtype=torch.float32, device=dev) if mu is not None else None
        g_lv = torch.empty_like(g_mu) if mu is not None else None
        if tail is not None:
            if unit_grad and ra_ is None and rb_ is None and mu_ is not None and gc is not None:
                try:
                    ops.class_tail(state.prec, B, tail.h0, tail.head, site, cw, mu_, lv_, beta, gamma, sums, gc, tail.d0_slice, g_mu, g_lv,
                                   beta_gamma_dev=beta_gamma_dev)
                    tail.done = True
                except ops.L.MMVAEArgError:
                    pass
            if not tail.done:
                lg_ = tail.logits(state.prec)
        if tail is None or not tail.done:
            ops.vae_loss(B, recon_a=ra_, a=a_, recon_b=rb_, b=b_, logits=lg_, site=site, class_weights=cw, mu=mu_, logvar=lv_,
                         beta=beta, gamma=gamma, sums=sums, g_a=ga, g_b=gb, grad_b_wrt_logit=True, g_c=gc, g_mu=g_mu, g_lv=g_lv,
                         beta_gamma_dev=beta_gamma_dev)
        if state.tail_riders and unit_grad:
            state.loss_tail = (sums, beta, gamma, out4, beta_gamma_dev)
        else:
            ops.loss_finalize(sums, beta, gamma, out4, beta_gamma_dev)
        if g_mu is None and state.logvar is not None:
            g_mu = torch.zeros(B, state.logvar.shape[1], dtype=torch.float32, device=dev)
            g_lv = torch.zeros_like(g_mu)
        state.loss_grads = engine.LossGrads(g_outs=g_outs, g_mu=g_mu, g_lv=g_lv, unit_grad=bool(unit_grad))
        pads = [t for t in (ra, rb, lg_real, mu, lv) if t is not None] + placeholders
        total = _LossHandleFn.apply(out4[0], state.loss_grads, *pads)
        return total, out4

    if fused is not None:
        raise RuntimeError("fused reconstruction loss: the loss terms are not all outputs of the one forward that computed it")
    if tail is not None:
        raise RuntimeError("fused class head: the loss terms are not all outputs of the one forward that left its logits to the loss")

    if sums is None:
        sums, out4 = ops.loss_workspace(dev)

    def spec(tensors):
        ga = torch.empty_like(ra_) if (need_grad and ra is not None and ra.requires_grad) else None
        gb = torch.empty_like(rb_) if (need_grad and rb is not None and rb.requires_grad) else None
        gc = torch.empty_like(lg_) if (need_grad and lg is not None and lg.requires_grad) else None
        gm = torch.empty_like(mu_) if (need_grad and mu is not None and mu.requires_grad) else None
        gl = torch.empty_like(lv_) if (need_grad and lv is not None and lv.requires_grad) else None
        ops.vae_loss(B, recon_a=ra_, a=a_, recon_b=rb_, b=b_, logits=lg_, site=site, class_weights=cw, mu=mu_, logvar=lv_,
                     beta=beta, gamma=gamma, sums=sums, g_a=ga, g_b=gb, grad_b_wrt_logit=False, g_c=gc, g_mu=gm, g_lv=gl,
                     beta_gamma_dev=beta_gamma_dev)
        ops.loss_finalize(sums, beta, gamma, out4, beta_gamma_dev)
        grads = []
        for t, g in ((ra, ga), (rb, gb), (lg, gc), (mu, gm), (lv, gl)):
            if t is not None:
                grads.append(g)
        return out4[0].clone(), grads

    inputs = [t for t in (ra, rb, lg, mu, lv) if t is not None]
    total = _LossGeneralFn.apply(spec, *inputs)
    return total, out4


def read_losses(out5):
    vals = out5.tolist()
    if vals[4] != 0.0:
        raise RuntimeError(f"vae_loss: {int(vals[4])} class index(es) in `site` outside [0, n_classes)")
    return vals[:4]


class ReparamFn(torch.autograd.Function):

    @staticmethod
    def forward(ctx, mu, logvar):
        if not (mu.is_cuda and logvar.is_cuda):
            raise RuntimeError(f"reparameterize: the MI355X path needs CUDA/HIP tensors (got {mu.device}); there is no CPU fallback")
        if mu.dim() != 2 or mu.shape != logvar.shape:
            raise RuntimeError(f"reparameterize: expected two (B, L) tensors, got {tuple(mu.shape)} and {tuple(logvar.shape)}")
        B, Ld = mu.shape
        heads = torch.cat([mu.detach().float(), logvar.detach().float()], dim=1).contiguous()
        eps = engine.GLOBAL_NOISE.draw(B, [], Ld, mu.device)[1]
        mu_o, lv_o = torch.empty_like(heads[:, :Ld]).contiguous(), torch.empty_like(heads[:, :Ld]).contiguous()
        z = torch.empty(B, Ld, dtype=torch.float32, device=mu.device)
        with ops.pinned_stream():
            ops.fuse_reparam_fwd(B, Ld, heads, None, None, None, eps, mu_o, lv_o, z)
        ctx.save_for_backward(eps, lv_o)
        return z

    @staticmethod
    def backward(ctx, g):
        eps, lv = ctx.saved_tensors
        B, Ld = lv.shape
# ... 116 lines not shown
```

### vae-los-angeles_amd/mmvae/graphs.py

```python
import torch

from . import engine, ops
from . import functional as F_


class GraphedTrainStep:
    KINDS = ("multimodal", "dna2rna", "rna2dna", "dna2rna_ae", "rna2dna_ae")

    def __init__(self, model, optimizer, a=None, b=None, site=None, beta=1e-3, gamma=1.0, class_weights=None, warmup=3, reduce=None,
                 preserve_state=False, kind="multimodal", dataset=None, batch_size=None, overlap=True):
        if kind not in self.KINDS:
            raise ValueError(f"kind must be one of {self.KINDS}")
        self.kind = kind
        self.dataset = dataset
        if dataset is not None:
            if batch_size is None:
                raise ValueError("dataset= needs batch_size=")
            dA, dB, dS = dataset
            if not dA.is_cuda:
                raise RuntimeError("GraphedTrainStep needs CUDA/HIP tensors; there is no CPU fallback")
            dev = dA.device
            a, b = (ops.zeros_bf16_rows(batch_size, t.shape[1], dev) if ops.is_bf16_rows(t)
                    else torch.empty((batch_size,) + tuple(t.shape[1:]), dtype=t.dtype, device=dev) for t in (dA, dB))
            site = torch.empty(batch_size, dtype=torch.int64, device=dev)
            self.index = torch.arange(batch_size, dtype=torch.int64, device=dev)
        if not a.is_cuda:
            raise RuntimeError("GraphedTrainStep needs CUDA/HIP tensors; there is no CPU fallback")
        self.model, self.optimizer = model, optimizer
        self.a, self.b, self.site = a, b, site
        self.beta, self.gamma, self.class_weights = float(beta), float(gamma), class_weights
        self.hyper = torch.tensor([self.beta, self.gamma], dtype=torch.float32, device=a.device)
        self.optimizer.device_lr(True)
        self.warmup = warmup
        self.reduce = reduce
        self.overlap = bool(overlap) and reduce is not None
        self.preserve_state = preserve_state
        self.graph = self.graph_opt = None
        self._one = torch.ones((), dtype=torch.float32, device=a.device)
        self.recapture()

    def set_beta(self, beta, gamma=None):
        gamma = self.gamma if gamma is None else float(gamma)
        if float(beta) != self.beta or gamma != self.gamma:
            self.beta, self.gamma = float(beta), gamma
            self.hyper.copy_(torch.tensor([self.beta, self.gamma], dtype=torch.float32), non_blocking=False)

    def set_indices(self, idx):
        self.index.copy_(idx, non_blocking=True)

    def _forward_loss(self):
        if self.dataset is not None:
            dA, dB, dS = self.dataset
            with ops.pinned_stream():
                ops.gather_rows([(dA, self.a), (dB, self.b), (dS, self.site)], self.index, dA.shape[0])
        g = self.model._graph()
        try:
            g.tail_riders = True
            if self.kind == "multimodal":
                g.fused_recon = [self.a, self.b, None]
                g.defer_class_head = True
                ra, rb, rc, mu, lv = self.model(a=self.a, b=self.b, site=self.site)
                terms = {"a": (ra, self.a), "b": (rb, self.b), "c": (rc, self.site), "kl": (mu, lv)}
            elif self.kind == "dna2rna":
                g.fused_recon = [self.a]
                rec, mu, lv = self.model(dna=self.b, site=self.site)
                terms = {"a": (rec, self.a), "kl": (mu, lv)}
            elif self.kind == "dna2rna_ae":
                g.fused_recon = [self.a]
                terms = {"a": (self.model(dna=self.b, site=self.site)[0], self.a)}
            elif self.kind == "rna2dna_ae":
                g.fused_recon = [self.b]
                terms = {"b": (self.model(rna=self.a, site=self.site)[0], self.b)}
            else:
                g.fused_recon = [self.b]
                rec, mu, lv = self.model(rna=self.a, site=self.site)
                terms = {"b": (rec, self.b), "kl": (mu, lv)}
        finally:
            g.fused_recon = None
            g.defer_class_head = False
            g.tail_riders = False
        if self.kind.endswith("_ae"):
            return F_.fused_loss(terms, 0.0, self.gamma, None, unit_grad=True)
        return F_.fused_loss(terms, self.beta, self.gamma, self.class_weights, unit_grad=True, beta_gamma_dev=self.hyper)

    def run_eager(self):
        return self._step()

    def _step(self):
        out4 = self._fwd_bwd()
        self.optimizer.step()
        return out4

    def _fwd_bwd(self):
        total, out4 = self._forward_loss()
        self.optimizer.zero_grad(set_to_none=True)
        total.backward(self._one)
        return out4

    def _flat_grads(self):
        ps = [p for p in self.model._graph().param_list() if p.grad is not None]
        lo = min(p.grad.data_ptr() for p in ps)
        hi = max(p.grad.data_ptr() + p.grad.numel() * 4 for p in ps)
        first = next(p for p in ps if p.grad.data_ptr() == lo)
        n = (hi - lo) // 4
        if n != sum(p.grad.numel() for p in ps):
            raise RuntimeError("gradients are not one contiguous arena")
        return torch.as_strided(first.grad, (n,), (1,))

    def recapture(self):
        self.model.train()
        g = self.model._graph()
        sync, g.grad_sync = g.grad_sync, (None if self.reduce is not None else g.grad_sync)
        try:
            snap = None
            if self.preserve_state:
                if self.warmup < 1:
                    raise ValueError("preserve_state needs at least one (undone) warm-up step")
                dev = self.a.device
                snap = ({k: v.clone() for k, v in self.model.state_dict().items()}, self.optimizer.snapshot(),
                        engine.GLOBAL_NOISE.state_dict(dev))
            side = torch.cuda.Stream()
            side.wait_stream(torch.cuda.current_stream())
            with torch.cuda.stream(side):
                for _ in range(self.warmup):
                    if self.reduce is None:
                        self._step()
                    else:
                        self._fwd_bwd()
                        self.reduce(self._flat_grads())
                        self.optimizer.step()
            torch.cuda.current_stream().wait_stream(side)
            torch.cuda.synchronize()
            if snap is not None:
                with torch.no_grad():
                    cur = self.model.state_dict()
                    for k, v in snap[0].items():
                        cur[k].copy_(v)
                self.optimizer.restore(snap[1])
                engine.GLOBAL_NOISE.load_state_dict(snap[2], self.a.device)
                torch.cuda.synchronize()
            self.graph = torch.cuda.CUDAGraph()
            self.graph_mid = None
            if self.reduce is None:
                with torch.cuda.graph(self.graph):
                    self.out4 = self._step()
            else:
                if self.overlap:
                    self._capture_split(g)
                else:
                    with torch.cuda.graph(self.graph):
                        self.out4 = self._fwd_bwd()
                self.flat = self._flat_grads()
                self.graph_opt = torch.cuda.CUDAGraph()
                with torch.cuda.graph(self.graph_opt, pool=self.graph.pool()):
                    self.optimizer.step()
            self.optimizer.note_captured_step()
        finally:
            g.grad_sync = sync
        return self

    def _capture_split(self, g):
        outer = self
# ... 72 lines not shown
```

### vae-los-angeles_amd/mmvae/ops.py

```python
import ctypes as C
from collections import namedtuple

import torch

from . import _lib as L
from ._lib import (F32, BF16, PREC_F32, PREC_BF16, PRO_NONE, PRO_BN_RELU_DROP, PRO_BN_BWD_APPLY, EPI_STORE, EPI_RELU_MASK,
                   EPI_BN_BWD, EPI_LOSS_MSE, EPI_LOSS_BCE_LOGIT, ACT_NONE, ACT_RELU, ACT_SIGMOID, TILE)

DROP_P = 0.1
BN_EPS, BN_MOMENTUM = 1e-5, 0.1


class KernelProbe:

    def __init__(self, only=None):
        self.records = {}
        self.only = only

    def wants(self, tag):
        return tag is not None and (self.only is None or tag in self.only)

    def begin(self):
        ev = torch.cuda.Event(enable_timing=True)
        ev.record(torch.cuda.current_stream())
# ... 518 lines not shown
        nbytes += enc.heads.K * (enc.y.element_size() + (enc.prologue[2] is not None))
    a.latent = latent.data_ptr()
    return a, B * nbytes


def ae_latent_fwd(prec, B, Ld, enc, table, site, latent, z, first, h0):
    if tuple(latent.shape) != (B, Ld) or not latent.is_contiguous() or latent.dtype != torch.float32:
        raise ValueError(f"ae_latent_fwd: latent must be contiguous fp32 ({B}, {Ld}), got {tuple(latent.shape)} / {latent.stride()}")
    a, nbytes = ae_latent_fwd_args(prec, B, Ld, enc, table, site, latent, z, first, h0)
    with stream_span("ae_latent.fwd", nbytes):
        L.check(L.load().mmvae_ae_latent_fwd(C.byref(a), _stream()), "mmvae_ae_latent_fwd")


def loss_workspace(device):
    buf = torch.zeros(5 * 8 + 5 * 4 + 4, dtype=torch.uint8, device=device)
    return buf[:40].view(torch.float64), buf[40:60].view(torch.float32)


def vae_loss(B, *, recon_a=None, a=None, recon_b=None, b=None, logits=None, site=None, class_weights=None,
             mu=None, logvar=None, beta=1e-3, gamma=1.0, sums=None, g_a=None, g_b=None, grad_b_wrt_logit=False,
             g_c=None, g_mu=None, g_lv=None, beta_gamma_dev=None):
    x = L.LossArgs()
    x.B = B
    if recon_a is not None:
        x.A, x.recon_a, x.a, x.ld_ra, x.ld_a, x.a_dtype = recon_a.shape[1], recon_a.data_ptr(), a.data_ptr(), _ld(recon_a), _ld(a), _dt(a)
    if recon_b is not None:
        x.D, x.recon_b, x.b, x.ld_rb, x.ld_b, x.b_dtype = recon_b.shape[1], recon_b.data_ptr(), b.data_ptr(), _ld(recon_b), _ld(b), _dt(b)
    if logits is not None:
        x.S, x.logits, x.ld_logits, x.site, x.class_weights = logits.shape[1], logits.data_ptr(), _ld(logits), site.data_ptr(), _p(class_weights)
    if mu is not None:
        x.L, x.mu, x.logvar = mu.shape[1], mu.data_ptr(), logvar.data_ptr()
    x.beta, x.gamma, x.sums = beta, gamma, sums.data_ptr()
    if g_a is not None:
        x.g_a, x.g_a_dtype, x.ld_ga = g_a.data_ptr(), _dt(g_a), _ld(g_a)
    if g_b is not None:
        x.g_b, x.g_b_dtype, x.ld_gb, x.grad_b_wrt_logit = g_b.data_ptr(), _dt(g_b), _ld(g_b), int(grad_b_wrt_logit)
    if g_c is not None:
        x.g_c, x.ld_gc = g_c.data_ptr(), _ld(g_c)
    x.g_mu, x.g_lv = _p(g_mu), _p(g_lv)
    x.beta_gamma_dev = _p(beta_gamma_dev)
    assert sums.dtype == torch.float64 and sums.numel() >= 5

    def nbytes():
        n = 0
        for pred, tgt, g in ((recon_a, a, g_a), (recon_b, b, g_b), (logits, None, g_c)):
            if pred is not None:
                n += B * pred.shape[1] * (4 + (4 if tgt is None else tgt.element_size())) + (0 if g is None else B * pred.shape[1] * g.element_size())
        if mu is not None:
            n += B * mu.shape[1] * 4 * (2 + (g_mu is not None) + (g_lv is not None))
        return n
    with stream_span("vae_loss", nbytes):
        L.check(L.load().mmvae_vae_loss(C.byref(x), _stream()), "mmvae_vae_loss")


def class_tail_fits(prec, S, hidden, Ld, ldh0, ldd0):
    return L.load().mmvae_class_tail_fits(prec, S, hidden, Ld, ldh0, ldd0) == 0


def class_tail_args(prec, B, h0, head, site, class_weights, mu, logvar, beta, gamma, sums, g_c, d0, g_mu, g_lv, beta_gamma_dev=None):
    a = L.ClassTailArgs()
    a.prec, a.B, a.S, a.L, a.hidden = prec, B, head.N, mu.shape[1], head.K
    a.h0, a.ldh0 = _mat(h0, "h0").data_ptr(), _ld(h0)
    a.w, a.ldw, a.wt, a.ldwt, a.bias = head.w.data_ptr(), head.w.stride(0), head.wt.data_ptr(), head.wt.stride(0), _p(head.bias)
    a.site, a.class_weights = site.data_ptr(), _p(class_weights)
    a.mu, a.logvar = mu.data_ptr(), logvar.data_ptr()
    a.beta, a.gamma, a.beta_gamma_dev, a.sums = beta, gamma, _p(beta_gamma_dev), sums.data_ptr()
    a.g_c, a.ld_gc = _mat(g_c, "g_c").data_ptr(), _ld(g_c)
    a.d0, a.ldd0 = _mat(d0, "d0").data_ptr(), _ld(d0)
    a.g_mu, a.g_lv = g_mu.data_ptr(), g_lv.data_ptr()
    nbytes = B * (2 * head.K * h0.element_size() + 8 + 4 * head.N + 16 * mu.shape[1])
    return a, nbytes


def class_tail(prec, B, h0, head, site, class_weights, mu, logvar, beta, gamma, sums, g_c, d0, g_mu, g_lv, beta_gamma_dev=None):
    for t in (mu, logvar, g_mu, g_lv):
        if tuple(t.shape) != (B, mu.shape[1]) or not t.is_contiguous() or t.dtype != torch.float32:
            raise ValueError(f"class_tail: mu / logvar / g_mu / g_lv must be contiguous fp32 ({B}, L), got {tuple(t.shape)} / {t.stride()}")
    assert sums.dtype == torch.float64 and sums.numel() >= 5 and site.dtype == torch.int64 and site.is_contiguous()
    a, nbytes = class_tail_args(prec, B, h0, head, site, class_weights, mu, logvar, beta, gamma, sums, g_c, d0, g_mu, g_lv, beta_gamma_dev)
    with stream_span("class_tail", nbytes):
        L.check(L.load().mmvae_class_tail(C.byref(a), _stream()), "mmvae_class_tail")


GROUP_MOMENTS_MAX_G = TILE


def group_moments_fits(prec, B, G, N, K, act=ACT_NONE, with_std=False, lda=None, ldw=None):
    lda = ceil_to(K, 8) if lda is None else lda
    ldw = ceil_to(K, 64) if ldw is None else ldw
    return L.load().mmvae_gemm_nt_group_moments_fits(prec, B, G, N, K, act, int(with_std), lda, ldw) == 0


def gemm_nt_group_moments(prec, a, pl_w, N, K, G, mean, std=None, bias=None, act=ACT_NONE):
    what = "gemm_nt_group_moments"
    a = _operand(a, "a", what, dtypes=None)
    if G < 1 or a.shape[0] % G:
        raise ValueError(f"{what}: a has {a.shape[0]} rows, not a multiple of G = {G}")
    B, dev = a.shape[0] // G, a.device
    pl_w = _operand(pl_w, "w", what, dtypes=None, dev=dev)
    mean = _operand(mean, "mean", what, dtypes=(torch.float32,), rows=B, dev=dev)
    if std is not None:
        std = _operand(std, "std", what, dtypes=(torch.float32,), rows=B, dev=dev)
    if mean.shape[1] < N or (std is not None and std.shape[1] < N) or a.shape[1] < K:
        raise ValueError(f"{what}: a needs >= {K} columns, mean / std >= {N}")
    if N < 1 or pl_w.shape[0] < ceil_to(N, TILE) or pl_w.shape[1] < K:
        raise ValueError(f"{what}: w must be a prepared operand of at least ({ceil_to(max(N, 1), TILE)}, {K}), got {tuple(pl_w.shape)}")
    if a.dtype != torch.bfloat16 or pl_w.dtype != torch.bfloat16:
        raise L.MMVAEArgError(f"{what} failed: dtype not supported for this precision")
    g = L.GroupMomentsArgs()
    g.prec, g.B, g.G, g.N, g.K, g.act = prec, B, G, N, K, act
    g.a, g.lda = a.data_ptr(), _ld(a)
    g.w, g.ldw, g.bias = pl_w.data_ptr(), pl_w.stride(0), _p(bias)
    g.mean, g.ld_mean = mean.data_ptr(), _ld(mean)
    g.std, g.ld_std = _p(std), _ld0(std)
    with stream_span(what, B * G * K * 2 + N * K * 2 + B * N * 4 * (1 + (std is not None))):
        L.check(L.load().mmvae_gemm_nt_group_moments(C.byref(g), _stream()), "mmvae_gemm_nt_group_moments")
    return mean, std


def loss_finalize(sums, beta, gamma, out5, beta_gamma_dev=None):
    assert out5.numel() >= 5
    L.check(L.load().mmvae_loss_finalize(sums.data_ptr(), beta, gamma, _p(beta_gamma_dev), out5.data_ptr(), _stream()), "mmvae_loss_finalize")


def sigmoid_bwd(g, p, out):
    L.check(L.load().mmvae_sigmoid_bwd(g.shape[0], g.shape[1], g.data_ptr(), _ld(g), p.data_ptr(), _ld(p), out.data_ptr(),
                                       _dt(out), _ld(out), _stream()), "mmvae_sigmoid_bwd")


def scale_many(tensors, scale):
    ts = [t for t in tensors if t is not None]
    for i in range(0, len(ts), 8):
        chunk = ts[i:i + 8]
        items = (L.ScaleItem * len(chunk))(*[L.ScaleItem(t.data_ptr(), t.numel(), _dt(t), 0) for t in chunk])
        L.check(L.load().mmvae_scale_many(items, len(chunk), scale.data_ptr(), _stream()), "mmvae_scale_many")


def scale_if_needed(x, scale):
    L.check(L.load().mmvae_scale_if_needed(x.data_ptr(), _dt(x), x.numel(), scale.data_ptr(), _stream()), "mmvae_scale_if_needed")


def noise(mask, eps, keep_prob, seed, offset, offset_dev=None, advance=False):
    n_mask = 0 if mask is None else mask.numel()
    n_eps = 0 if eps is None else eps.numel()
    if advance:
        assert offset_dev is not None and offset_dev.numel() == L.CTR_COPIES and offset_dev.dtype == torch.int64
    with stream_span("noise", n_mask + 4 * n_eps):
        L.check(L.load().mmvae_noise(_p(mask), n_mask, keep_prob, _p(eps), n_eps, seed, offset, _p(offset_dev), int(advance), _stream()), "mmvae_noise")
    return (n_mask + 15) // 16 * 4 + (n_eps + 3) // 4


def step_head(noise_args=None, prep=None, zero=(), table_args=None):
    a = L.StepHeadArgs()
    nbytes = 0
    if noise_args is not None:
        mask, eps, keep_prob, seed, offset, offset_dev, advance = noise_args
        a.mask, a.n_mask = _p(mask), 0 if mask is None else mask.numel()
        a.eps, a.n_eps = _p(eps), 0 if eps is None else eps.numel()
        if advance:
            assert offset_dev is not None and offset_dev.numel() == L.CTR_COPIES and offset_dev.dtype == torch.int64
        a.keep_prob, a.seed, a.offset, a.offset_dev, a.advance = keep_prob, seed, offset, _p(offset_dev), int(advance)
        nbytes += a.n_mask + 4 * a.n_eps
    if prep is not None:
        a.prep_items, a.n_prep = prep.table.data_ptr(), prep.n
        nbytes += prep.nbytes()
    zero = [z for z in zero if z is not None and z.numel()]
# ... 604 lines not shown
```

Baseline: 55.01 million.

## Fuse class head loss and backward into latent forward kernel

Pulls the class-tail body into a shared header and adds a new latent_class_fwd kernel that runs the classifier head, cross-entropy loss and gradient, the KL gradient, and the d0 slice inside the latent/stem forward pass. The training graph promises the loss hyperparameters ahead of time so the forward can run the class head, and the later fused_loss reuses the precomputed g_c, g_mu and g_lv instead of launching class_tail. This is meant to remove a separate kernel launch and the re-read of h0, mu and logvar. In exchange it adds a promise and validation mechanism that raises an error if the loss call does not match what was promised.

```diff
diff --git a/include/mmvae_hip.h b/include/mmvae_hip.h
--- a/include/mmvae_hip.h
+++ b/include/mmvae_hip.h
@@ -193,6 +193,24 @@
 int mmvae_class_tail_fits(int32_t prec, int32_t S, int32_t hidden, int32_t L, int64_t ldh0, int64_t ldd0);
 
 typedef struct {
+    int32_t S, hidden;
+    const void* w; int64_t ldw; const void* wt; int64_t ldwt; const float* bias;
+    const float* class_weights;
+    float beta, gamma; const float* beta_gamma_dev;
+    double* sums;
+    float* g_c; int64_t ld_gc;
+    void* d0; int64_t ldd0;
+    float* g_mu; float* g_lv;
+} mmvae_class_head;
+typedef struct {
+    mmvae_latent_fwd_args latent;
+    mmvae_class_head cls;
+    int32_t stem_col;
+} mmvae_latent_class_fwd_args;
+int mmvae_latent_class_fwd(const mmvae_latent_class_fwd_args* args, void* stream);
+int mmvae_latent_class_fits(int32_t prec, int32_t S, int32_t hidden, int32_t L, int32_t N_stem, int32_t stem_col, int64_t ldh0, int64_t ldd0);
+
+typedef struct {
     int32_t prec, B, G, N, K, act;
     const void* a; int64_t lda;
     const void* w; int64_t ldw; const float* bias;
diff --git a/vae-los-angeles_amd/csrc/class_slab.h b/vae-los-angeles_amd/csrc/class_slab.h
--- /dev/null
+++ b/vae-los-angeles_amd/csrc/class_slab.h
@@ -0,0 +1,177 @@
+#pragma once
+#include "common.h"
+#include "mmvae_hip.h"
+#include "loss_terms.h"
+#include "wave_slab.h"
+
+namespace mm {
+
+constexpr int CT_WAVES = 8, CT_THREADS = 64 * CT_WAVES;
+constexpr int CT_SP = 32;
+constexpr int CT_HID = 64;
+constexpr int CT_KU = 6;
+constexpr int CT_WROW = 2 * CT_HID + 16;
+constexpr int CT_TROW = 2 * CT_SP + 16;
+constexpr int CT_XLD = CT_SP + 4;
+constexpr int CT_OFF_WT = CT_SP * CT_WROW;
+constexpr int CT_OFF_BIAS = CT_OFF_WT + CT_HID * CT_TROW;
+constexpr int CT_OFF_CW = CT_OFF_BIAS + CT_SP * 4;
+constexpr int CT_OFF_RED = CT_OFF_CW + CT_SP * 4;
+constexpr int CT_OFF_SCR = CT_OFF_RED + CT_WAVES * 3 * 8;
+constexpr int CT_SCR_E = 16 * CT_XLD * 4;
+static_assert(CT_OFF_SCR % 16 == 0 && CT_SCR_E % 16 == 0, "16-byte LDS vectors");
+
+struct ClassHead {
+    int B, S, L;
+    const bf16* w; long ldw; const bf16* wt; long ldwt; const float* bias;
+    const long long* site; const float* cw;
+    float beta, gamma; const float* bg; double* sums;
+    float* gc; long ldgc; bf16* d0; long ldd; float* gmu; float* glv;
+};
+
+struct ClassLds { unsigned char* ct; float* sx; float* sexp; unsigned char* sg; };
+
+template <int NT>
+__device__ __forceinline__ void class_stage(unsigned char* ct, const ClassHead& a, int tid) {
+    float* const sbias = (float*)(ct + CT_OFF_BIAS);
+    float* const scw = (float*)(ct + CT_OFF_CW);
+    stage_rows<NT>(ct, CT_WROW, a.w, a.ldw, CT_SP, 8, tid, EpiCols<false>::wrow);
+    stage_rows<NT>(ct + CT_OFF_WT, CT_TROW, a.wt, a.ldwt, CT_HID, 4, tid, EpiCols<true>::wrow);
+    if (tid < CT_SP) {
+        sbias[tid] = (a.bias && tid < a.S) ? a.bias[tid] : 0.f;
+        scw[tid] = (a.cw && tid < a.S) ? a.cw[tid] : 1.f;
+    }
+}
+
+__device__ __forceinline__ void class_slab_head(const ClassLds& s, const ClassHead& a, int slab, const bf16x8 (&hv)[2], long long yl, float gamma,
+                                                int lane, double& dcls, float& nbad) {
+    const int li = lane & 15, lg = lane >> 4;
+    const int S = a.S;
+    const float* const sbias = (const float*)(s.ct + CT_OFF_BIAS);
+    const float* const scw = (const float*)(s.ct + CT_OFF_CW);
+    float* const sx = s.sx;
+    float* const sexp = s.sexp;
+    unsigned char* const sg = s.sg;
+    const int vpr = S >> 2;
+    const int row = slab * 16 + li;
+    const bool rok = row < a.B;
+
+    f32x4 x[2];
+#pragma unroll
+    for (int n = 0; n < 2; ++n) {
+        f32x4 acc = {0.f, 0.f, 0.f, 0.f};
+#pragma unroll
+        for (int j = 0; j < 2; ++j) {
+            const bf16x8 wf = *(const bf16x8*)(s.ct + (16 * n + li) * CT_WROW + (4 * j + lg) * 16);
+            Mma<bf16>::mma(acc, wf, hv[j]);
+        }
+        x[n] = acc + *(const f32x4*)(sbias + 16 * n + 4 * lg);
+    }
+    float m = -INFINITY;
+#pragma unroll
+    for (int n = 0; n < 2; ++n)
+#pragma unroll
+        for (int j = 0; j < 4; ++j) {
+            if (16 * n + 4 * lg + j >= S) x[n][j] = -INFINITY;
+            m = fmaxf(m, x[n][j]);
+        }
+    m = fmaxf(m, __shfl_xor(m, 16, 64));
+    m = fmaxf(m, __shfl_xor(m, 32, 64));
+    f32x4 e[2];
+#pragma unroll
+    for (int n = 0; n < 2; ++n) {
+#pragma unroll
+        for (int j = 0; j < 4; ++j) e[n][j] = (16 * n + 4 * lg + j < S) ? ce_exp(x[n][j], m) : 0.f;
+        *(f32x4*)(sx + li * CT_XLD + 16 * n + 4 * lg) = x[n];
+        *(f32x4*)(sexp + li * CT_XLD + 16 * n + 4 * lg) = e[n];
+    }
+    wave_lds_sync();
+    float se = 0.f;
+#pragma unroll
+    for (int c = 0; c < CT_SP / 4; ++c) {
+        const f32x4 v = *(const f32x4*)(sexp + li * CT_XLD + 4 * c);
+#pragma unroll
+        for (int j = 0; j < 4; ++j) se += v[j];
+    }
+    const CeLabel lb = ce_label(yl, S, scw);
+    const float xy = sx[li * CT_XLD + lb.y];
+    if (lg == 0 && rok) {
+        dcls += (double)ce_term(lb.w, m, se, xy);
+        if (lb.bad) nbad += 1.f;
+    }
+    const float gw = gamma * lb.w;
+    f32x4 g[2];
+#pragma unroll
+    for (int n = 0; n < 2; ++n)
+#pragma unroll
+        for (int j = 0; j < 4; ++j) {
+            const int c = 16 * n + 4 * lg + j;
+            g[n][j] = c < S ? ce_grad(gw, e[n][j], se, c == lb.y) : 0.f;
+        }
+    wave_lds_sync();
+#pragma unroll
+    for (int n = 0; n < 2; ++n) {
+        *(f32x4*)(sx + li * CT_XLD + 16 * n + 4 * lg) = g[n];
+        const bf16x4 gb = {(bf16)g[n][0], (bf16)g[n][1], (bf16)g[n][2], (bf16)g[n][3]};
+        *(bf16x4*)(sg + li * CT_TROW + (16 * n + 4 * lg) * 2) = gb;
+    }
+    wave_lds_sync();
+#pragma unroll
+    for (int it = 0; it < 2; ++it) {
+        const int v = lane + 64 * it;
+        const int r = v / vpr, c4 = v - r * vpr;
+        if (v < 16 * vpr && slab * 16 + r < a.B)
+            *(f32x4*)(a.gc + (long)(slab * 16 + r) * a.ldgc + 4 * c4) = *(const f32x4*)(sx + r * CT_XLD + 4 * c4);
+    }
+    const bf16x8 gf = *(const bf16x8*)(sg + li * CT_TROW + lg * 16);
+    f32x4 acc[4];
+#pragma unroll
+    for (int q = 0; q < 4; ++q) {
+        const bf16x8 wf = *(const bf16x8*)(s.ct + CT_OFF_WT + (16 * q + li) * CT_TROW + lg * 16);
+        acc[q] = f32x4{0.f, 0.f, 0.f, 0.f};
+        Mma<bf16>::mma(acc[q], wf, gf);
+    }
+    uint32_t pk[2][4];
+#pragma unroll
+    for (int h = 0; h < 2; ++h) {
+#pragma unroll
+        for (int qd = 0; qd < 4; ++qd) {
+            const f32x4 v = qd < 2 ? acc[2 * h] : acc[2 * h + 1];
+            const int e0 = 2 * qd;
+            const float o0 = (float)hv[h][e0] > 0.f ? v[2 * (qd & 1)] : 0.f;
+            const float o1 = (float)hv[h][e0 + 1] > 0.f ? v[2 * (qd & 1) + 1] : 0.f;
+            const bf16x2 t = {(bf16)o0, (bf16)o1};
+            pk[h][qd] = __builtin_bit_cast(uint32_t, t);
+        }
+    }
+    SWAP_HALVES(pk, li < 8, st0, st1);
+    const int rbase = slab * 16 + (li & 7);
+    bf16* const crow = line_col(a.d0 + (long)rbase * a.ldd, li, lg);
+    if (rbase < a.B) *(uint4*)crow = uint4{st0[0], st0[1], st0[2], st0[3]};
+    if (rbase + 8 < a.B) *(uint4*)(crow + 8 * a.ldd) = uint4{st1[0], st1[1], st1[2], st1[3]};
+}
+
+__device__ __forceinline__ void class_kl_elem(const ClassHead& a, int idx, float mu, float lv, float beta, double& dkl) {
+    float gm, gl;
+    dkl += (double)kl_elem(mu, lv, beta, gm, gl);
+    a.gmu[idx] = gm; a.glv[idx] = gl;
+}
+
+__device__ __forceinline__ void class_sums(unsigned char* ct, double* sums, int tid, double dcls, double dkl, float nbad) {
+    double* const red = (double*)(ct + CT_OFF_RED);
+    const int lane = tid & 63, wid = tid >> 6;
+    const double vc = wave_sum_f64(dcls), vk = wave_sum_f64(dkl);
+    const float vb = wave_sum(nbad);
+    if (lane == 0) { red[wid * 3] = vc; red[wid * 3 + 1] = vk; red[wid * 3 + 2] = (double)vb; }
+    __syncthreads();
+    if (tid < 3) {
+        double v = 0.0;
+#pragma unroll
+        for (int w = 0; w < CT_WAVES; ++w) v += red[w * 3 + tid];
+        if (v != 0.0) unsafeAtomicAdd(sums + 2 + tid, v);
+    }
+}
+
+int class_head_check(const mmvae_class_head& a, const int64_t* site, int32_t prec, int32_t B, int32_t L, int64_t ldh0, ClassHead& k);
+
+}
diff --git a/vae-los-angeles_amd/csrc/class_tail.hip b/vae-los-angeles_amd/csrc/class_tail.hip
--- a/vae-los-angeles_amd/csrc/class_tail.hip
+++ b/vae-los-angeles_amd/csrc/class_tail.hip
@@ -1,60 +1,38 @@
 #include "common.h"
 #include "mmvae_hip.h"
-#include "loss_terms.h"
-#include "wave_slab.h"
+#include "class_slab.h"
 
 namespace mm {
 
-constexpr int CT_WAVES = 8, CT_THREADS = 64 * CT_WAVES;
-constexpr int CT_SP = 32;
-constexpr int CT_HID = 64;
-constexpr int CT_KU = 6;
-constexpr int CT_WROW = 2 * CT_HID + 16;
-constexpr int CT_TROW = 2 * CT_SP + 16;
-constexpr int CT_XLD = CT_SP + 4;
-constexpr int CT_OFF_WT = CT_SP * CT_WROW;
-constexpr int CT_OFF_BIAS = CT_OFF_WT + CT_HID * CT_TROW;
-constexpr int CT_OFF_CW = CT_OFF_BIAS + CT_SP * 4;
-constexpr int CT_OFF_RED = CT_OFF_CW + CT_SP * 4;
-constexpr int CT_OFF_SCR = CT_OFF_RED + CT_WAVES * 3 * 8;
-constexpr int CT_SCR_E = 16 * CT_XLD * 4;
 constexpr int CT_SCR_G = 2 * CT_SCR_E;
 constexpr int CT_SCR = CT_SCR_G + 16 * CT_TROW;
 constexpr int CT_LDS = CT_OFF_SCR + CT_WAVES * CT_SCR;
-static_assert(CT_OFF_SCR % 16 == 0 && CT_SCR % 16 == 0 && CT_SCR_E % 16 == 0, "16-byte LDS vectors");
+static_assert(CT_SCR % 16 == 0, "16-byte LDS vectors");
 
 struct CtArgs {
-    int B, S, L, nslabs;
-    const bf16* h0; long ldh; const bf16* w; long ldw; const bf16* wt; long ldwt; const float* bias;
-    const long long* site; const float* cw; const float* mu; const float* lv;
-    float beta, gamma; const float* bg; double* sums;
-    float* gc; long ldgc; bf16* d0; long ldd; float* gmu; float* glv;
+    ClassHead c; int nslabs;
+    const bf16* h0; long ldh; const float* mu; const float* lv;
 };
 
 __global__ __launch_bounds__(CT_THREADS) void class_tail_kernel(const CtArgs a) {
     extern __shared__ __attribute__((aligned(16))) unsigned char smem[];
     const int tid = threadIdx.x, lane = tid & 63, wid = tid >> 6;
     const int li = lane & 15, lg = lane >> 4;
-    float* const sbias = (float*)(smem + CT_OFF_BIAS);
-    float* const scw = (float*)(smem + CT_OFF_CW);
-    double* const red = (double*)(smem + CT_OFF_RED);
     unsigned char* const scr = smem + CT_OFF_SCR + wid * CT_SCR;
-    float* const sx = (float*)scr;
-    float* const sexp = (float*)(scr + CT_SCR_E);
-    unsigned char* const sg = scr + CT_SCR_G;
-    float beta = a.beta, gamma = a.gamma;
-    if (a.bg) { beta = a.bg[0]; gamma = a.bg[1]; }
-    const int S = a.S, L = a.L, total = a.B * L;
+    const ClassLds lds = {smem, (float*)scr, (float*)(scr + CT_SCR_E), scr + CT_SCR_G};
+    float beta = a.c.beta, gamma = a.c.gamma;
+    if (a.c.bg) { beta = a.c.bg[0]; gamma = a.c.bg[1]; }
+    const int L = a.c.L, total = a.c.B * L;
 
     bf16x8 hn[2];
     long long yn = 0;
     float mun[CT_KU] = {}, lvn[CT_KU] = {};
     auto fetch = [&](int slab) __attribute__((always_inline)) {
-        const int row = min(slab * 16 + li, a.B - 1);
+        const int row = min(slab * 16 + li, a.c.B - 1);
         const bf16* hp = a.h0 + (long)row * a.ldh + 8 * lg;
         hn[0] = *(const bf16x8*)hp;
         hn[1] = *(const bf16x8*)(hp + 32);
-        yn = a.site[row];
+        yn = a.c.site[row];
 #pragma unroll
         for (int i = 0; i < CT_KU; ++i) {
             if (64 * i >= 16 * L) break;
@@ -67,17 +45,11 @@
     int slab = blockIdx.x * CT_WAVES + wid;
     if (slab < a.nslabs) fetch(slab);
 
-    stage_rows<CT_THREADS>(smem, CT_WROW, a.w, a.ldw, CT_SP, 8, tid, EpiCols<false>::wrow);
-    stage_rows<CT_THREADS>(smem + CT_OFF_WT, CT_TROW, a.wt, a.ldwt, CT_HID, 4, tid, EpiCols<true>::wrow);
-    if (tid < CT_SP) {
-        sbias[tid] = (a.bias && tid < S) ? a.bias[tid] : 0.f;
-        scw[tid] = (a.cw && tid < S) ? a.cw[tid] : 1.f;
-    }
+    class_stage<CT_THREADS>(smem, a.c, tid);
     __syncthreads();
 
     double dcls = 0.0, dkl = 0.0;
     float nbad = 0.f;
-    const int vpr = S >> 2;
     for (; slab < a.nslabs; slab += nw) {
         const bf16x8 hv[2] = {hn[0], hn[1]};
         const long long yl = yn;
@@ -85,126 +57,35 @@
 #pragma unroll
         for (int i = 0; i < CT_KU; ++i) { mu[i] = mun[i]; lv[i] = lvn[i]; }
         if (slab + nw < a.nslabs) fetch(slab + nw);
-        const int row = slab * 16 + li;
-        const bool rok = row < a.B;
-
-        f32x4 x[2];
-#pragma unroll
-        for (int n = 0; n < 2; ++n) {
-            f32x4 acc = {0.f, 0.f, 0.f, 0.f};
-#pragma unroll
-            for (int j = 0; j < 2; ++j) {
-                const bf16x8 wf = *(const bf16x8*)(smem + (16 * n + li) * CT_WROW + (4 * j + lg) * 16);
-                Mma<bf16>::mma(acc, wf, hv[j]);
-            }
-            x[n] = acc + *(const f32x4*)(sbias + 16 * n + 4 * lg);
-        }
-        float m = -INFINITY;
-#pragma unroll
-        for (int n = 0; n < 2; ++n)
-#pragma unroll
-            for (int j = 0; j < 4; ++j) {
-                if (16 * n + 4 * lg + j >= S) x[n][j] = -INFINITY;
-                m = fmaxf(m, x[n][j]);
-            }
-        m = fmaxf(m, __shfl_xor(m, 16, 64));
-        m = fmaxf(m, __shfl_xor(m, 32, 64));
-        f32x4 e[2];
-#pragma unroll
-        for (int n = 0; n < 2; ++n) {
-#pragma unroll
-            for (int j = 0; j < 4; ++j) e[n][j] = (16 * n + 4 * lg + j < S) ? ce_exp(x[n][j], m) : 0.f;
-            *(f32x4*)(sx + li * CT_XLD + 16 * n + 4 * lg) = x[n];
-            *(f32x4*)(sexp + li * CT_XLD + 16 * n + 4 * lg) = e[n];
-        }
-        wave_lds_sync();
-        float se = 0.f;
-#pragma unroll
-        for (int c = 0; c < CT_SP / 4; ++c) {
-            const f32x4 v = *(const f32x4*)(sexp + li * CT_XLD + 4 * c);
-#pragma unroll
-            for (int j = 0; j < 4; ++j) se += v[j];
-        }
-        const CeLabel lb = ce_label(yl, S, scw);
-        const float xy = sx[li * CT_XLD + lb.y];
-        if (lg == 0 && rok) {
-            dcls += (double)ce_term(lb.w, m, se, xy);
-            if (lb.bad) nbad += 1.f;
-        }
-        const float gw = gamma * lb.w;
-        f32x4 g[2];
-#pragma unroll
-        for (int n = 0; n < 2; ++n)
-#pragma unroll
-            for (int j = 0; j < 4; ++j) {
-                const int c = 16 * n + 4 * lg + j;
-                g[n][j] = c < S ? ce_grad(gw, e[n][j], se, c == lb.y) : 0.f;
-            }
-        wave_lds_sync();
-#pragma unroll
-        for (int n = 0; n < 2; ++n) {
-            *(f32x4*)(sx + li * CT_XLD + 16 * n + 4 * lg) = g[n];
-            const bf16x4 gb = {(bf16)g[n][0], (bf16)g[n][1], (bf16)g[n][2], (bf16)g[n][3]};
-            *(bf16x4*)(sg + li * CT_TROW + (16 * n + 4 * lg) * 2) = gb;
-        }
-        wave_lds_sync();
-#pragma unroll
-        for (int it = 0; it < 2; ++it) {
-            const int v = lane + 64 * it;
-            const int r = v / vpr, c4 = v - r * vpr;
-            if (v < 16 * vpr && slab * 16 + r < a.B)
-                *(f32x4*)(a.gc + (long)(slab * 16 + r) * a.ldgc + 4 * c4) = *(const f32x4*)(sx + r * CT_XLD + 4 * c4);
-        }
-        const bf16x8 gf = *(const bf16x8*)(sg + li * CT_TROW + lg * 16);
-        f32x4 acc[4];
-#pragma unroll
-        for (int q = 0; q < 4; ++q) {
-            const bf16x8 wf = *(const bf16x8*)(smem + CT_OFF_WT + (16 * q + li) * CT_TROW + lg * 16);
-            acc[q] = f32x4{0.f, 0.f, 0.f, 0.f};
-            Mma<bf16>::mma(acc[q], wf, gf);
-        }
-        uint32_t pk[2][4];
-#pragma unroll
-        for (int h = 0; h < 2; ++h) {
-#pragma unroll
-            for (int qd = 0; qd < 4; ++qd) {
-                const f32x4 v = qd < 2 ? acc[2 * h] : acc[2 * h + 1];
-                const int e0 = 2 * qd;
-                const float o0 = (float)hv[h][e0] > 0.f ? v[2 * (qd & 1)] : 0.f;
-                const float o1 = (float)hv[h][e0 + 1] > 0.f ? v[2 * (qd & 1) + 1] : 0.f;
-                const bf16x2 t = {(bf16)o0, (bf16)o1};
-                pk[h][qd] = __builtin_bit_cast(uint32_t, t);
-            }
-        }
-        SWAP_HALVES(pk, li < 8, st0, st1);
-        const int rbase = slab * 16 + (li & 7);
-        bf16* const crow = line_col(a.d0 + (long)rbase * a.ldd, li, lg);
-        if (rbase < a.B) *(uint4*)crow = uint4{st0[0], st0[1], st0[2], st0[3]};
-        if (rbase + 8 < a.B) *(uint4*)(crow + 8 * a.ldd) = uint4{st1[0], st1[1], st1[2], st1[3]};
+        class_slab_head(lds, a.c, slab, hv, yl, gamma, lane, dcls, nbad);
 
 #pragma unroll
         for (int i = 0; i < CT_KU; ++i) {
             if (64 * i >= 16 * L) break;
             const int idx = slab * 16 * L + lane + 64 * i;
-            if (lane + 64 * i < 16 * L && idx < total) {
-                float gm, gl;
-                dkl += (double)kl_elem(mu[i], lv[i], beta, gm, gl);
-                a.gmu[idx] = gm; a.glv[idx] = gl;
-            }
+            if (lane + 64 * i < 16 * L && idx < total) class_kl_elem(a.c, idx, mu[i], lv[i], beta, dkl);
         }
         wave_lds_sync();
     }
 
-    const double vc = wave_sum_f64(dcls), vk = wave_sum_f64(dkl);
-    const float vb = wave_sum(nbad);
-    if (lane == 0) { red[wid * 3] = vc; red[wid * 3 + 1] = vk; red[wid * 3 + 2] = (double)vb; }
-    __syncthreads();
-    if (tid < 3) {
-        double v = 0.0;
-#pragma unroll
-        for (int w = 0; w < CT_WAVES; ++w) v += red[w * 3 + tid];
-        if (v != 0.0) unsafeAtomicAdd(a.sums + 2 + tid, v);
-    }
+    class_sums(smem, a.c.sums, tid, dcls, dkl, nbad);
+}
+
+int class_head_check(const mmvae_class_head& a, const int64_t* site, int32_t prec, int32_t B, int32_t L, int64_t ldh0, ClassHead& k) {
+    { const int rc = mmvae_class_tail_fits(prec, a.S, a.hidden, L, ldh0, a.ldd0); if (rc) return rc; }
+    const long wide = L > a.S ? L : a.S;
+    if (B <= 0 || (long)B * wide >= (1L << 31)) return MMVAE_ERR_ARG;
+    if (!a.w || !a.wt || !a.bias || !site || !a.sums || !a.g_c || !a.d0 || !a.g_mu || !a.g_lv) return MMVAE_ERR_ARG;
+    if (((uintptr_t)a.d0 & 127) || ((uintptr_t)a.w & 15) || ((uintptr_t)a.wt & 15)) return MMVAE_ERR_ARG;
+    if (a.ldw % 8 || a.ldw < CT_HID || a.ldwt % 8 || a.ldwt < CT_SP) return MMVAE_ERR_ARG;
+    if (((uintptr_t)a.g_c & 15) || a.ld_gc % 4 || a.ld_gc < a.S) return MMVAE_ERR_ARG;
+    k = ClassHead{};
+    k.B = B; k.S = a.S; k.L = L;
+    k.w = (const bf16*)a.w; k.ldw = a.ldw; k.wt = (const bf16*)a.wt; k.ldwt = a.ldwt;
+    k.bias = a.bias; k.site = (const long long*)site; k.cw = a.class_weights;
+    k.beta = a.beta; k.gamma = a.gamma; k.bg = a.beta_gamma_dev; k.sums = a.sums;
+    k.gc = a.g_c; k.ldgc = a.ld_gc; k.d0 = (bf16*)a.d0; k.ldd = a.ldd0; k.gmu = a.g_mu; k.glv = a.g_lv;
+    return 0;
 }
 
 }
@@ -221,19 +102,12 @@
 extern "C" int mmvae_class_tail(const mmvae_class_tail_args* a, void* stream) {
     using namespace mm;
     if (!a) return MMVAE_ERR_ARG;
-    { const int rc = mmvae_class_tail_fits(a->prec, a->S, a->hidden, a->L, a->ldh0, a->ldd0); if (rc) return rc; }
-    const long wide = a->L > a->S ? a->L : a->S;
-    if (a->B <= 0 || (long)a->B * wide >= (1L << 31)) return MMVAE_ERR_ARG;
-    if (!a->h0 || !a->w || !a->wt || !a->bias || !a->site || !a->mu || !a->logvar || !a->sums || !a->g_c || !a->d0 || !a->g_mu || !a->g_lv)
-        return MMVAE_ERR_ARG;
-    if (((uintptr_t)a->h0 & 15) || ((uintptr_t)a->d0 & 127) || ((uintptr_t)a->w & 15) || ((uintptr_t)a->wt & 15)) return MMVAE_ERR_ARG;
-    if (a->ldw % 8 || a->ldw < CT_HID || a->ldwt % 8 || a->ldwt < CT_SP) return MMVAE_ERR_ARG;
-    if (((uintptr_t)a->g_c & 15) || a->ld_gc % 4 || a->ld_gc < a->S) return MMVAE_ERR_ARG;
+    const mmvae_class_head h = {a->S, a->hidden, a->w, a->ldw, a->wt, a->ldwt, a->bias, a->class_weights, a->beta, a->gamma, a->beta_gamma_dev,
+                                a->sums, a->g_c, a->ld_gc, a->d0, a->ldd0, a->g_mu, a->g_lv};
     CtArgs k{};
-    k.B = a->B; k.S = a->S; k.L = a->L; k.nslabs = (a->B + 15) / 16;
-    k.h0 = (const bf16*)a->h0; k.ldh = a->ldh0; k.w = (const bf16*)a->w; k.ldw = a->ldw; k.wt = (const bf16*)a->wt; k.ldwt = a->ldwt;
-    k.bias = a->bias; k.site = (const long long*)a->site; k.cw = a->class_weights; k.mu = a->mu; k.lv = a->logvar;
-    k.beta = a->beta; k.gamma = a->gamma; k.bg = a->beta_gamma_dev; k.sums = a->sums;
-    k.gc = a->g_c; k.ldgc = a->ld_gc; k.d0 = (bf16*)a->d0; k.ldd = a->ldd0; k.gmu = a->g_mu; k.glv = a->g_lv;
+    { const int rc = class_head_check(h, a->site, a->prec, a->B, a->L, a->ldh0, k.c); if (rc) return rc; }
+    if (!a->h0 || !a->mu || !a->logvar || ((uintptr_t)a->h0 & 15)) return MMVAE_ERR_ARG;
+    k.nslabs = (a->B + 15) / 16;
+    k.h0 = (const bf16*)a->h0; k.ldh = a->ldh0; k.mu = a->mu; k.lv = a->logvar;
     return launch_lds<class_tail_kernel>(dim3(persistent_grid(k.nslabs, CT_WAVES)), dim3(CT_THREADS), CT_LDS, (hipStream_t)stream, k);
 }
diff --git a/vae-los-angeles_amd/csrc/common.h b/vae-los-angeles_amd/csrc/common.h
--- a/vae-los-angeles_amd/csrc/common.h
+++ b/vae-los-angeles_amd/csrc/common.h
@@ -165,6 +165,7 @@
     int class_tail_on = 1;
     int step_head_on = 1;
     int ae_latent_on = 1;
+    int latent_class_on = 1;
     int tn_riders_on = 1;
 };
 inline Tuning g_tuning;
diff --git a/vae-los-angeles_amd/csrc/gemm_nt.hip b/vae-los-angeles_amd/csrc/gemm_nt.hip
--- a/vae-los-angeles_amd/csrc/gemm_nt.hip
+++ b/vae-los-angeles_amd/csrc/gemm_nt.hip
@@ -334,6 +334,7 @@
     case 13: t.step_head_on = value; return 0;
     case 14: t.tn_riders_on = value; return 0;
     case 15: t.ae_latent_on = value; return 0;
+    case 17: t.latent_class_on = value; return 0;
     }
     return MMVAE_ERR_ARG;
 }
diff --git a/vae-los-angeles_amd/csrc/latent.hip b/vae-los-angeles_amd/csrc/latent.hip
--- a/vae-los-angeles_amd/csrc/latent.hip
+++ b/vae-los-angeles_amd/csrc/latent.hip
@@ -3,6 +3,7 @@
 #include "gemm_src.h"
 #include "fuse_math.h"
 #include "wave_slab.h"
+#include "class_slab.h"
 
 namespace mm {
 
@@ -23,6 +24,13 @@
 constexpr int LAT_SCR_Z = 16 * LAT_SUMLD * 4;
 constexpr int LAT_SCR = LAT_SCR_Z + 16 * LAT_SROW;
 constexpr int LAT_LDS = LAT_OFF_SCR + LAT_WAVES * LAT_SCR;
+constexpr int LATC_SCR_Z = 2 * CT_SCR_E;
+constexpr int LATC_SCR = LATC_SCR_Z + 16 * LAT_SROW;
+constexpr int LATC_OFF_CT = LAT_OFF_SCR + LAT_WAVES * LATC_SCR;
+constexpr int LATC_LDS = LATC_OFF_CT + CT_OFF_SCR;
+static_assert(LATC_SCR_Z >= LAT_SCR_Z && 16 * CT_TROW <= CT_SCR_E && LATC_SCR % 16 == 0 && LATC_OFF_CT % 16 == 0 && LATC_LDS <= 160 * 1024,
+              "the class form's images: over the heads image, 16-byte LDS vectors, one CU's LDS");
+static_assert(CT_WAVES == LAT_WAVES && CT_KU == LAT_FU, "class_slab.h: the same waves and the same element order of a slab's [16][L] block");
 
 struct LatEnc { SrcBnReluDrop<bf16> src; const bf16* w; long ldw; const float* bias; int nk; };
 struct LatArgs {
@@ -35,8 +43,12 @@
     int nslabs;
 };
 
-template <bool DET>
-__global__ __launch_bounds__(LAT_THREADS) void latent_fwd_kernel(const LatArgs a) {
+struct LatCls { ClassHead c; int p; };
+struct LatNoCls {};
+
+template <bool DET, bool CLS = false>
+__global__ __launch_bounds__(LAT_THREADS) void latent_fwd_kernel(const LatArgs a, const std::conditional_t<CLS, LatCls, LatNoCls> cl) {
+    static_assert(!(DET && CLS), "the class form is the VAE's");
     typedef SrcBnReluDrop<bf16>::Raw Raw;
     extern __shared__ __attribute__((aligned(16))) unsigned char smem[];
     const int tid = threadIdx.x, lane = tid & 63, wid = tid >> 6;
@@ -44,15 +56,18 @@
     float* const aux = (float*)(smem + LAT_OFF_AUX);
     float* const sbias = (float*)(smem + LAT_OFF_BIAS);
     float* const stab = (float*)(smem + LAT_OFF_TAB);
-    unsigned char* const scr = smem + LAT_OFF_SCR + wid * LAT_SCR;
+    unsigned char* const scr = smem + LAT_OFF_SCR + wid * (CLS ? LATC_SCR : LAT_SCR);
     float* const ssum = (float*)scr;
-    unsigned char* const sz = scr + LAT_SCR_Z;
+    unsigned char* const sz = scr + (CLS ? LATC_SCR_Z : LAT_SCR_Z);
     const int L = a.L, L2 = DET ? a.L : 2 * a.L;
     const bool any_enc = a.e[0].nk + a.e[1].nk > 0;
 
     int fr[LAT_FU], fl[LAT_FU];
-#pragma unroll
-    for (int i = 0; i < LAT_FU; ++i) { const int x = lane + 64 * i; fr[i] = x / L; fl[i] = x - fr[i] * L; }
+    auto lane_consts = [&](int ln) __attribute__((always_inline)) {
+#pragma unroll
+        for (int i = 0; i < LAT_FU; ++i) { const int x = ln + 64 * i; fr[i] = x / L; fl[i] = x - fr[i] * L; }
+    };
+    if constexpr (!CLS) lane_consts(lane);
     const int zcpr = (int)(a.ldz >> 3), zr = lane / zcpr, zc = lane - zr * zcpr;
     const float inv_n = 1.f / (float)a.n_mod;
     const int total = a.B * L;
@@ -60,6 +75,7 @@
     Raw raw[2][LAT_NK];
     float eps_r[LAT_FU] = {};
     long long site_r[LAT_FU] = {};
+    long long yn = 0;
     auto fetch = [&](int slab) __attribute__((always_inline)) {
         const int row = slab * 16 + li;
 #pragma unroll
@@ -74,7 +90,9 @@
                 eps_r[i] = a.eps[idx];
             }
         }
-        if (a.table) {
+        if constexpr (CLS) {
+            yn = a.site[min(slab * 16 + li, a.B - 1)];
+        } else if (a.table) {
 #pragma unroll
             for (int i = 0; i < LAT_FU; ++i) site_r[i] = a.site[min(slab * 16 + fr[i], a.B - 1)];
         }
@@ -96,7 +114,15 @@
     for (int c = tid; c < a.ns; c += LAT_THREADS) sbias[2 * LAT_HN + c] = a.bs ? a.bs[c] : 0.f;
     if (a.table) for (int i = tid; i < a.S * L2; i += LAT_THREADS) stab[i] = a.table[i];
     for (int i = lane; i < 16 * LAT_SROW / 16; i += 64) ((uint4*)sz)[i] = uint4{0u, 0u, 0u, 0u};
+    if constexpr (CLS) class_stage<LAT_THREADS>(smem + LATC_OFF_CT, cl.c, tid);
     __syncthreads();
+
+    double dcls = 0.0, dkl = 0.0;
+    float nbad = 0.f, beta = 0.f, gamma = 0.f;
+    if constexpr (CLS) {
+        beta = cl.c.beta; gamma = cl.c.gamma;
+        if (cl.c.bg) { beta = cl.c.bg[0]; gamma = cl.c.bg[1]; }
+    }
 
     for (; slab < a.nslabs; slab += nw) {
         f32x4 hs[3];
@@ -131,8 +157,16 @@
         long long st[LAT_FU];
 #pragma unroll
         for (int i = 0; i < LAT_FU; ++i) { ep[i] = eps_r[i]; st[i] = site_r[i]; }
+        const long long yl = yn;
         if (slab + nw < a.nslabs) fetch(slab + nw);
         wave_lds_sync();
+        if constexpr (CLS) {
+            int lane_f = lane;
+            asm volatile("" : "+v"(lane_f));
+            lane_consts(lane_f);
+#pragma unroll
+            for (int i = 0; i < LAT_FU; ++i) st[i] = __shfl(yl, fr[i], 64);
+        }
 
 #pragma unroll
         for (int i = 0; i < LAT_FU; ++i) {
@@ -165,7 +199,10 @@
             }
             const float zf = fuse_reparam_elem(mu, lv, a.n_mod, inv_n, ep[i]);
             const int idx = slab * 16 * L + lane + 64 * i;
-            if (idx < total) { a.mu[idx] = mu; a.logvar[idx] = lv; }
+            if (idx < total) {
+                a.mu[idx] = mu; a.logvar[idx] = lv;
+                if constexpr (CLS) class_kl_elem(cl.c, idx, mu, lv, beta, dkl);
+            }
             ((bf16*)sz)[r * (LAT_SROW / 2) + l] = (bf16)zf;
         }
         wave_lds_sync();
@@ -177,7 +214,7 @@
         const int rbase = slab * 16 + (li & 7);
         bf16* const crow = line_col(a.h0 + (long)rbase * a.ldh0, li, lg);
         const bool ok0 = rbase < a.B, ok1 = rbase + 8 < a.B;
-        for (int p = 0; p < (a.ns >> 6); ++p) {
+        auto stem_block = [&](int p, uint32_t (&pk)[2][4]) __attribute__((always_inline)) {
             f32x4 acc[4];
 #pragma unroll
             for (int q = 0; q < 4; ++q) {
@@ -185,7 +222,6 @@
                 acc[q] = f32x4{0.f, 0.f, 0.f, 0.f};
                 Mma<bf16>::mma(acc[q], wf, zf8);
             }
-            uint32_t pk[2][4];
 #pragma unroll
             for (int h = 0; h < 2; ++h) {
                 const float* bp = sbias + 2 * LAT_HN + 64 * p + 32 * h + 8 * lg;
@@ -201,9 +237,26 @@
             SWAP_HALVES(pk, lowl, st0, st1);
             if (ok0) *(uint4*)(crow + 64 * p) = uint4{st0[0], st0[1], st0[2], st0[3]};
             if (ok1) *(uint4*)(crow + 8 * a.ldh0 + 64 * p) = uint4{st1[0], st1[1], st1[2], st1[3]};
+        };
+        if constexpr (CLS) {
+            uint32_t pk[2][4];
+            stem_block(cl.p, pk);
+            const bf16x8 hv[2] = {__builtin_bit_cast(bf16x8, pk[0]), __builtin_bit_cast(bf16x8, pk[1])};
+            wave_lds_sync();
+            int lane_c = lane, wid_c = wid;
+            asm volatile("" : "+v"(lane_c), "+v"(wid_c));
+            unsigned char* const scr_c = smem + LAT_OFF_SCR + wid_c * LATC_SCR;
+            const ClassLds lds = {smem + LATC_OFF_CT, (float*)scr_c, (float*)(scr_c + CT_SCR_E), scr_c + CT_SCR_E};
+            class_slab_head(lds, cl.c, slab, hv, yl, gamma, lane_c, dcls, nbad);
+        }
+        for (int p = 0; p < (a.ns >> 6); ++p) {
+            if constexpr (CLS) { if (p == cl.p) continue; }
+            uint32_t pk[2][4];
+            stem_block(p, pk);
         }
         wave_lds_sync();
     }
+    if constexpr (CLS) class_sums(smem + LATC_OFF_CT, cl.c.sums, tid, dcls, dkl, nbad);
 }
 
 static int lat_enc(const mmvae_latent_enc& e, int B, LatEnc& o) {
@@ -224,7 +277,8 @@
 }
 
 template <bool DET, typename A>
-static int latent_check_launch(const A& a, bool own_ok, const mmvae_latent_enc& enc_a, const mmvae_latent_enc* enc_b, LatArgs& k, void* stream) {
+static int latent_check_launch(const A& a, bool own_ok, const mmvae_latent_enc& enc_a, const mmvae_latent_enc* enc_b, LatArgs& k, void* stream,
+                               const LatCls* cls = nullptr) {
     if (a.prec != MMVAE_PREC_BF16) return MMVAE_ERR_DTYPE;
     if (a.B <= 0 || a.L <= 0 || (long)a.B * a.L >= (1L << 31) || !own_ok) return MMVAE_ERR_ARG;
     if (!a.z || !a.w_stem || !a.h0) return MMVAE_ERR_ARG;
@@ -242,7 +296,11 @@
     k.ws = (const bf16*)a.w_stem; k.ldws = a.ldw_stem; k.bs = a.bias_stem; k.ns = a.N_stem;
     k.h0 = (bf16*)a.h0; k.ldh0 = a.ldh0;
     k.nslabs = (a.B + 15) / 16;
-    return launch_lds<latent_fwd_kernel<DET>>(dim3(persistent_grid(k.nslabs, LAT_WAVES)), dim3(LAT_THREADS), LAT_LDS, (hipStream_t)stream, k);
+    const dim3 grid(persistent_grid(k.nslabs, LAT_WAVES));
+    if constexpr (!DET) {
+        if (cls) return launch_lds<latent_fwd_kernel<false, true>>(grid, dim3(LAT_THREADS), LATC_LDS, (hipStream_t)stream, k, *cls);
+    }
+    return launch_lds<latent_fwd_kernel<DET>>(grid, dim3(LAT_THREADS), LAT_LDS, (hipStream_t)stream, k, LatNoCls{});
 }
 
 }
@@ -256,6 +314,30 @@
     return latent_check_launch<false>(*a, own_ok, a->enc_a, &a->enc_b, k, stream);
 }
 
+extern "C" int mmvae_latent_class_fits(int32_t prec, int32_t S, int32_t hidden, int32_t L, int32_t N_stem, int32_t stem_col, int64_t ldh0, int64_t ldd0) {
+    using namespace mm;
+    if (!g_tuning.latent_on || !g_tuning.latent_class_on) return MMVAE_ERR_ARG;
+    { const int rc = mmvae_class_tail_fits(prec, S, hidden, L, ldh0, ldd0); if (rc) return rc; }
+    if (2 * L > LAT_HN || N_stem < 64 || N_stem % 64 || N_stem > LAT_NS || ldh0 % 64 || ldh0 < N_stem) return MMVAE_ERR_ARG;
+    if (stem_col < 0 || stem_col % 64 || stem_col + CT_HID > N_stem) return MMVAE_ERR_ARG;
+    return 0;
+}
+
+extern "C" int mmvae_latent_class_fwd(const mmvae_latent_class_fwd_args* ac, void* stream) {
+    using namespace mm;
+    if (!ac) return MMVAE_ERR_ARG;
+    const mmvae_latent_fwd_args* a = &ac->latent;
+    if (a->prec != MMVAE_PREC_BF16) return MMVAE_ERR_DTYPE;
+    { const int rc = mmvae_latent_class_fits(a->prec, ac->cls.S, ac->cls.hidden, a->L, a->N_stem, ac->stem_col, a->ldh0, ac->cls.ldd0); if (rc) return rc; }
+    LatCls cls{};
+    { const int rc = class_head_check(ac->cls, a->site, a->prec, a->B, a->L, a->ldh0, cls.c); if (rc) return rc; }
+    cls.p = ac->stem_col / 64;
+    const bool own_ok = 2 * a->L <= LAT_HN && a->eps && a->mu && a->logvar && (!a->table || (long)a->S * 2 * a->L <= LAT_MAXTAB);
+    LatArgs k{};
+    k.eps = a->eps; k.mu = a->mu; k.logvar = a->logvar;
+    return latent_check_launch<false>(*a, own_ok, a->enc_a, &a->enc_b, k, stream, &cls);
+}
+
 extern "C" int mmvae_ae_latent_fwd(const mmvae_ae_latent_fwd_args* a, void* stream) {
     using namespace mm;
     if (!a || !g_tuning.ae_latent_on) return MMVAE_ERR_ARG;
diff --git a/vae-los-angeles_amd/mmvae/_lib.py b/vae-los-angeles_amd/mmvae/_lib.py
--- a/vae-los-angeles_amd/mmvae/_lib.py
+++ b/vae-los-angeles_amd/mmvae/_lib.py
@@ -139,6 +139,21 @@
                 ("g_c", vp), ("ld_gc", i64),
                 ("d0", vp), ("ldd0", i64),
                 ("g_mu", vp), ("g_lv", vp)]
+
+
+class ClassHead(C.Structure):
+    _fields_ = [("S", i32), ("hidden", i32),
+                ("w", vp), ("ldw", i64), ("wt", vp), ("ldwt", i64), ("bias", vp),
+                ("class_weights", vp),
+                ("beta", f32), ("gamma", f32), ("beta_gamma_dev", vp),
+                ("sums", vp),
+                ("g_c", vp), ("ld_gc", i64),
+                ("d0", vp), ("ldd0", i64),
+                ("g_mu", vp), ("g_lv", vp)]
+
+
+class LatentClassFwdArgs(C.Structure):
+    _fields_ = [("latent", LatentFwdArgs), ("cls", ClassHead), ("stem_col", i32)]
 
 
 class GroupMomentsArgs(C.Structure):
@@ -311,6 +326,8 @@
     "mmvae_ae_latent_fwd": [C.POINTER(AELatentFwdArgs), vp],
     "mmvae_class_tail": [C.POINTER(ClassTailArgs), vp],
     "mmvae_class_tail_fits": [i32, i32, i32, i32, i64, i64],
+    "mmvae_latent_class_fwd": [C.POINTER(LatentClassFwdArgs), vp],
+    "mmvae_latent_class_fits": [i32, i32, i32, i32, i32, i32, i64, i64],
     "mmvae_gemm_nt_group_moments": [C.POINTER(GroupMomentsArgs), vp],
     "mmvae_gemm_nt_group_moments_fits": [i32, i32, i32, i32, i32, i32, i32, i64, i64],
     "mmvae_vae_loss": [C.POINTER(LossArgs), vp],
diff --git a/vae-los-angeles_amd/mmvae/engine.py b/vae-los-angeles_amd/mmvae/engine.py
--- a/vae-los-angeles_amd/mmvae/engine.py
+++ b/vae-los-angeles_amd/mmvae/engine.py
@@ -178,6 +178,21 @@
     armed: bool = False
 
 
+class ClassHeadLoss(NamedTuple):
+    beta: float
+    gamma: float
+    class_weights: Optional[torch.Tensor]
+    beta_gamma_dev: Optional[torch.Tensor]
+
+
+class ClassHeadResult(NamedTuple):
+    promise: ClassHeadLoss
+    sums: torch.Tensor
+    g_c: torch.Tensor
+    g_mu: torch.Tensor
+    g_lv: torch.Tensor
+
+
 @dataclass(slots=True, eq=False)
 class ClassTail:
     index: int
@@ -187,6 +202,7 @@
     d0_slice: torch.Tensor
     name: str
     done: bool = False
+    in_forward: Optional["ClassHeadResult"] = None
 
     def logits(self, prec):
         out = torch.empty(self.h0.shape[0], self.head.N, dtype=torch.float32, device=self.h0.device)
@@ -221,6 +237,7 @@
     loss_grads: Optional[LossGrads] = None
     class_tail: Optional[ClassTail] = None
     tail_riders: bool = False
+    step_head: bool = False
     loss_tail: Optional[tuple] = None
     consumed: bool = False
 
@@ -472,6 +489,7 @@
         self.grad_sync = None
         self.fused_recon = None
         self.defer_class_head = False
+        self.class_head_loss = None
         self.tail_riders = False
 
     def _late_decoder_params(self):
@@ -586,6 +604,7 @@
             table = table_args[-1]
         if want_bwd:
             state.zeros = zeros
+        state.step_head = head
         fuse_latent = self._fuses_latent(prec)
         if xa is not None:
             xa = _check_input(xa.reshape(xa.shape[0], -1) if self.flatten_a else xa, "a", self.enc_a.in_dim, prec)
@@ -618,7 +637,19 @@
         H0 = torch.empty(B, stem.N, dtype=act_dtype(prec), device=dev) if stem is not None else None
         if fused:
             try:
-                ops.latent_fwd(prec, B, Ld, heads_a, heads_b, table, site, eps, mu, logvar, z, stem, H0)
+                tail, cw = self._class_head_in_forward(prec, B, dev, H0, site, state)
+                if tail is not None:
+                    r = tail.in_forward
+                    try:
+                        ops.latent_class_fwd(prec, B, Ld, heads_a, heads_b, table, site, eps, mu, logvar, z, stem, H0,
+                                             tail.h0.storage_offset() - H0.storage_offset(),
+                                             tail.head, cw, r.promise.beta, r.promise.gamma, r.sums, r.g_c, tail.d0_slice,
+                                             r.g_mu, r.g_lv, beta_gamma_dev=r.promise.beta_gamma_dev)
+                        tail.done, state.class_tail = True, tail
+                    except L_.MMVAEArgError:
+                        tail = None
+                if tail is None:
+                    ops.latent_fwd(prec, B, Ld, heads_a, heads_b, table, site, eps, mu, logvar, z, stem, H0)
             except L_.MMVAEArgError:
                 fused = False
                 heads_a = self.enc_a.run_heads(prec, heads_a) if heads_a is not None else None
@@ -627,6 +658,28 @@
             ops.fuse_reparam_fwd(B, Ld, heads_a, heads_b, table, site, eps, mu, logvar, z)
         state.logvar = logvar.detach()
         return (mu, logvar), z, H0, fused, None
+
+    def _class_head_in_forward(self, prec, B, dev, H0, site, state):
+        promise, want, zeros = self.class_head_loss, self.fused_recon, state.zeros
+        if promise is None or not self.defer_class_head or want is None or not state.step_head or zeros is None or zeros.loss_ws is None:
+            return None, None
+        if not all((t is None) or self.decoders[i].can_fuse_loss(prec) for i, t in enumerate(want)) or all(t is None for t in want):
+            return None, None
+        i = self._class_tail_index(prec, H0, want, site)
+        if i is None:
+            return None, None
+        dec, stem = self.decoders[i], self.dec_stem
+        off, n0 = sum(d.linears[0].out_features for d in self.decoders[:i]), dec.linears[0].out_features
+        if not ops.latent_class_fits(prec, dec.pl[1].N, dec.pl[1].K, self.latent, stem.N, off, H0.stride(0), H0.stride(0)):
+            return None, None
+        cw = promise.class_weights
+        if cw is not None:
+            cw = cw.to(device=dev, dtype=torch.float32).contiguous()
+        D0 = torch.empty(B, stem.N, dtype=act_dtype(prec), device=dev)
+        g_mu = torch.empty(B, self.latent, dtype=torch.float32, device=dev)
+        res = ClassHeadResult(promise, zeros.loss_ws[0],
+                              torch.empty(B, dec.pl[1].N, dtype=torch.float32, device=dev), g_mu, torch.empty_like(g_mu))
+        return ClassTail(i, dec.pl[1], H0[:, off:off + n0], D0, D0[:, off:off + n0], dec.name, in_forward=res), cw
 
     def _decode(self, prec, B, dev, z, H0, stem_done, state, zeros, want_bwd, site, first0=None):
         stem = self.dec_stem
@@ -645,11 +698,16 @@
         want = self.fused_recon
         if want is not None and any(t is not None and self.decoders[i].can_fuse_loss(prec) for i, t in enumerate(want)):
             fused = state.fused = FusedRecon(*(zeros.loss_ws if want_bwd else ops.loss_workspace(dev)), {}, {})
-        tail_i = self._class_tail_index(prec, H0, want, site) if (self.defer_class_head and fused is not None and want_bwd) else None
+        ran = state.class_tail
+        tail_i = ran.index if ran is not None else \
+            self._class_tail_index(prec, H0, want, site) if (self.defer_class_head and fused is not None and want_bwd) else None
         for i in order:
             dec = self.decoders[i]
             tgt = want[i] if (fused is not None and want[i] is not None and dec.can_fuse_loss(prec)) else None
-            if i == tail_i:
+            if ran is not None and i == tail_i:
+                o = torch.empty(1, dtype=torch.float32, device=dev).expand(B, dec.out_dim)
+                acts = [z, firsts[i]]
+            elif i == tail_i:
                 D0 = torch.empty(B, stem.N, dtype=act_dtype(prec), device=dev)
                 off = sum(d.linears[0].out_features for d in self.decoders[:i])
                 state.class_tail = ClassTail(i, dec.pl[1], firsts[i], D0, D0[:, off:off + dec.linears[0].out_features], dec.name)
diff --git a/vae-los-angeles_amd/mmvae/functional.py b/vae-los-angeles_amd/mmvae/functional.py
--- a/vae-los-angeles_amd/mmvae/functional.py
+++ b/vae-los-angeles_amd/mmvae/functional.py
@@ -205,8 +205,16 @@
         rb = None
     tg = _tag_of(lg)
     tail = tg.state.class_tail if (tg is not None and tg.kind == "out") else None
-    if tail is not None and (tail.index != tg.index or tail.done):
+    if tail is not None and (tail.index != tg.index or (tail.done and tail.in_forward is None)):
         tail = None
+    ran = tail.in_forward if tail is not None else None
+    if ran is not None:
+        pr = ran.promise
+        if not (unit_grad and float(beta) == pr.beta and float(gamma) == pr.gamma and class_weights is pr.class_weights
+                and beta_gamma_dev is pr.beta_gamma_dev and mu is not None and site.data_ptr() == tg.state.site.data_ptr()
+                and need_grad and lg.requires_grad and tg.state.loss_grads is None):
+            raise RuntimeError("fused class head: the forward ran the class head for the loss its caller promised (VAEGraph.class_head_loss); "
+                               "this loss call differs from that promise")
     lg_real = lg
     if tail is not None:
         lg = None
@@ -244,12 +252,18 @@
         if rb is not None and rb.requires_grad:
             gb = torch.empty(B, ceil_to(rb.shape[1], 8), dtype=adt, device=dev)
             g_outs[_tag_of(rb).index] = gb
-        if lg_real is not None and lg_real.requires_grad:
+        if ran is not None:
+            if sums.data_ptr() != ran.sums.data_ptr() or ra_ is not None or rb_ is not None:
+                raise RuntimeError("fused class head: the loss terms are not all outputs of the one forward that ran the class head")
+            gc, g_mu, g_lv = ran.g_c, ran.g_mu, ran.g_lv
+            g_outs[_tag_of(lg_real).index] = gc
+        elif lg_real is not None and lg_real.requires_grad:
             gc = torch.empty(B, lg_real.shape[1], dtype=torch.float32, device=dev)
             g_outs[_tag_of(lg_real).index] = gc
-        g_mu = torch.empty(B, mu.shape[1], dtype=torch.float32, device=dev) if mu is not None else None
-        g_lv = torch.empty_like(g_mu) if mu is not None else None
-        if tail is not None:
+        if ran is None:
+            g_mu = torch.empty(B, mu.shape[1], dtype=torch.float32, device=dev) if mu is not None else None
+            g_lv = torch.empty_like(g_mu) if mu is not None else None
+        if tail is not None and ran is None:
             if unit_grad and ra_ is None and rb_ is None and mu_ is not None and gc is not None:
                 try:
                     ops.class_tail(state.prec, B, tail.h0, tail.head, site, cw, mu_, lv_, beta, gamma, sums, gc, tail.d0_slice, g_mu, g_lv,
diff --git a/vae-los-angeles_amd/mmvae/graphs.py b/vae-los-angeles_amd/mmvae/graphs.py
--- a/vae-los-angeles_amd/mmvae/graphs.py
+++ b/vae-los-angeles_amd/mmvae/graphs.py
@@ -59,6 +59,7 @@
             if self.kind == "multimodal":
                 g.fused_recon = [self.a, self.b, None]
                 g.defer_class_head = True
+                g.class_head_loss = engine.ClassHeadLoss(self.beta, self.gamma, self.class_weights, self.hyper)
                 ra, rb, rc, mu, lv = self.model(a=self.a, b=self.b, site=self.site)
                 terms = {"a": (ra, self.a), "b": (rb, self.b), "c": (rc, self.site), "kl": (mu, lv)}
             elif self.kind == "dna2rna":
@@ -78,6 +79,7 @@
         finally:
             g.fused_recon = None
             g.defer_class_head = False
+            g.class_head_loss = None
             g.tail_riders = False
         if self.kind.endswith("_ae"):
             return F_.fused_loss(terms, 0.0, self.gamma, None, unit_grad=True)
diff --git a/vae-los-angeles_amd/mmvae/ops.py b/vae-los-angeles_amd/mmvae/ops.py
--- a/vae-los-angeles_amd/mmvae/ops.py
+++ b/vae-los-angeles_amd/mmvae/ops.py
@@ -624,6 +624,40 @@
         L.check(L.load().mmvae_class_tail(C.byref(a), _stream()), "mmvae_class_tail")
 
 
+def latent_class_fits(prec, S, hidden, Ld, n_stem, stem_col, ldh0, ldd0):
+    return L.load().mmvae_latent_class_fits(prec, S, hidden, Ld, n_stem, stem_col, ldh0, ldd0) == 0
+
+
+def latent_class_fwd_args(prec, B, Ld, enc_a, enc_b, table, site, eps, mu, logvar, z, stem, h0,
+                          stem_col, head, class_weights, beta, gamma, sums, g_c, d0, g_mu, g_lv, beta_gamma_dev=None):
+    a = L.LatentClassFwdArgs()
+    a.latent, nbytes = latent_fwd_args(prec, B, Ld, enc_a, enc_b, table, site, eps, mu, logvar, z, stem, h0)
+    a.latent.site = site.data_ptr()
+    c = a.cls
+    c.S, c.hidden = head.N, head.K
+    c.w, c.ldw, c.wt, c.ldwt, c.bias = head.w.data_ptr(), head.w.stride(0), head.wt.data_ptr(), head.wt.stride(0), _p(head.bias)
+    c.class_weights = _p(class_weights)
+    c.beta, c.gamma, c.beta_gamma_dev, c.sums = beta, gamma, _p(beta_gamma_dev), sums.data_ptr()
+    c.g_c, c.ld_gc = _mat(g_c, "g_c").data_ptr(), _ld(g_c)
+    c.d0, c.ldd0 = _mat(d0, "d0").data_ptr(), _ld(d0)
+    c.g_mu, c.g_lv = g_mu.data_ptr(), g_lv.data_ptr()
+    a.stem_col = stem_col
+    nbytes += B * (8 * (table is None) + 4 * head.N + head.K * d0.element_size() + 8 * Ld)
+    return a, nbytes
+
+
+def latent_class_fwd(prec, B, Ld, enc_a, enc_b, table, site, eps, mu, logvar, z, stem, h0,
+                     stem_col, head, class_weights, beta, gamma, sums, g_c, d0, g_mu, g_lv, beta_gamma_dev=None):
+    for t in (eps, mu, logvar, g_mu, g_lv):
+        if tuple(t.shape) != (B, Ld) or not t.is_contiguous() or t.dtype != torch.float32:
+            raise ValueError(f"latent_class_fwd: eps / mu / logvar / g_mu / g_lv must be contiguous fp32 ({B}, {Ld}), got {tuple(t.shape)} / {t.stride()}")
+    assert sums.dtype == torch.float64 and sums.numel() >= 5 and site.dtype == torch.int64 and site.is_contiguous()
+    a, nbytes = latent_class_fwd_args(prec, B, Ld, enc_a, enc_b, table, site, eps, mu, logvar, z, stem, h0,
+                                      stem_col, head, class_weights, beta, gamma, sums, g_c, d0, g_mu, g_lv, beta_gamma_dev)
+    with stream_span("latent_class.fwd", nbytes):
+        L.check(L.load().mmvae_latent_class_fwd(C.byref(a), _stream()), "mmvae_latent_class_fwd")
+
+
 GROUP_MOMENTS_MAX_G = TILE
 
 
```

New measurement: 55.39 million (median of 6 runs). No clear change (+0.7%).
